# xXJSONDeruloXx/linux-fg

Hardware: AMD Instinct MI355X
Metric: interpolated frames/s, 1080p->4K RGBA8 (higher is better)
Workload: dtype f32 arithmetic on u8 RGBA (u8 in, u8 out; int8 motion vectors); 1 GPU; 1080p->2160p scale+motion(8,16)+interpolate; order=one call per stage, semantics=reference, frames_in_flight=3, content=translated (the motion stage's best case but `static`; see content_sweep), parallelism=one frame pair per GPU x1, gpu_max_hw_queues=4

## Files before the change

### include/linuxfg_hip.h

```cpp
#ifndef LINUXFG_HIP_H
#define LINUXFG_HIP_H

#include <stddef.h>
#include <stdint.h>

#ifdef __cplusplus
extern "C" {
#endif

#define LFG_ABI_VERSION 1

typedef enum lfg_status {
    LFG_OK = 0,
    LFG_ERR_INVALID = -1,
    LFG_ERR_DEVICE = -2,
    LFG_ERR_NOMEM = -3,
    LFG_ERR_UNSUPPORTED = -4
} lfg_status;

typedef enum lfg_format {
    LFG_FORMAT_RGBA8_UNORM = 0,
    LFG_FORMAT_MV_S8X2 = 1,
    LFG_FORMAT_MV_S16X2_Q2 = 2
} lfg_format;

typedef struct lfg_frame {
    void    *data;
    uint32_t width;
    uint32_t height;
    uint32_t pitch;
    uint32_t format;
    uint32_t owned;
    uint32_t reserved;
} lfg_frame;

typedef struct lfg_context lfg_context;
typedef struct lfg_ring lfg_ring;

typedef enum lfg_stage {
    LFG_STAGE_SCALE = 0,
    LFG_STAGE_MOTION = 1,
    LFG_STAGE_INTERPOLATE = 2,
    LFG_STAGE_COUNT = 3
} lfg_stage;


int         lfg_abi_version(void);
int         lfg_device_count(void);

int         lfg_context_create(int device_ordinal, lfg_context **out_ctx);
void        lfg_context_destroy(lfg_context *ctx);
int         lfg_context_set_stream(lfg_context *ctx, void *hip_stream);
void       *lfg_context_get_stream(lfg_context *ctx);
int         lfg_context_device(const lfg_context *ctx);
int         lfg_sync(lfg_context *ctx);

#define LFG_MAX_LANES 4
int         lfg_lanes(lfg_context *ctx, int count);
int         lfg_lane_count(const lfg_context *ctx);
int         lfg_lane_current(const lfg_context *ctx);
int         lfg_lane_select(lfg_context *ctx, int lane);
int         lfg_lane_mark(lfg_context *ctx);
int         lfg_lane_wait(lfg_context *ctx, int other);
int         lfg_lane_sync(lfg_context *ctx);
const char *lfg_last_error(const lfg_context *ctx);


int  lfg_frame_create(lfg_context *ctx, uint32_t width, uint32_t height, uint32_t format, lfg_frame *out);
void lfg_frame_destroy(lfg_context *ctx, lfg_frame *frame);
int  lfg_frame_wrap(void *device_ptr, uint32_t width, uint32_t height, uint32_t pitch, uint32_t format,
                    lfg_frame *out);
int  lfg_frame_copy(lfg_context *ctx, const lfg_frame *src, lfg_frame *dst);

int  lfg_staging_create(lfg_context *ctx, size_t bytes, void **out_host_ptr);
void lfg_staging_destroy(lfg_context *ctx, void *host_ptr);

int  lfg_frame_upload(lfg_context *ctx, lfg_frame *dst, const void *host, size_t bytes);
int  lfg_frame_download(lfg_context *ctx, const lfg_frame *src, void *host, size_t bytes);

int  lfg_ring_create(lfg_context *ctx, uint32_t slots, size_t slot_bytes, lfg_ring **out_ring);
void lfg_ring_destroy(lfg_ring *ring);
int  lfg_ring_acquire(lfg_ring *ring, void **out_host_ptr, uint32_t *out_slot);
int  lfg_ring_upload(lfg_ring *ring, uint32_t slot, lfg_frame *dst);
int  lfg_ring_download(lfg_ring *ring, uint32_t slot, const lfg_frame *src);
int  lfg_ring_wait(lfg_ring *ring, uint32_t slot);
int  lfg_ring_fence_slot(lfg_ring *ring, uint32_t slot);


int  lfg_scale(lfg_context *ctx, const lfg_frame *in, lfg_frame *out);
int  lfg_scale_last_kernel(const lfg_context *ctx);

int  lfg_motion(lfg_context *ctx, const lfg_frame *prev, const lfg_frame *curr, lfg_frame *mv,
                int block_size, float search_radius);

typedef enum lfg_motion_mode { LFG_MOTION_PREFILTERED = 0, LFG_MOTION_EXACT_ONLY = 1 } lfg_motion_mode;
int  lfg_set_motion_mode(lfg_context *ctx, int mode);
int  lfg_motion_last_stats(lfg_context *ctx, uint32_t *out_tiles, uint32_t *out_fallback_tiles,
                           double *out_mean_recorded);
int  lfg_motion_open_segments(lfg_context *ctx, uint32_t *out_open, uint32_t *out_segments);
int  lfg_motion_lean_stats(lfg_context *ctx, int *out_used, uint32_t *out_tiles, uint32_t *out_tiles_left);
int  lfg_motion_strip_stats(lfg_context *ctx, uint32_t *out_rows, uint32_t *out_columns);
int  lfg_motion_last_variant(const lfg_context *ctx);
int  lfg_motion_prediction_stats(const lfg_context *ctx, uint64_t *out_verdicts, uint64_t *out_lean_wrong,
                                 uint64_t *out_grid_wrong, uint64_t *out_second_pass_wrong);
int  lfg_motion_workspace_size(lfg_context *ctx, uint32_t width, uint32_t height, uint64_t *out_bytes);
int  lfg_motion_plan(const lfg_context *ctx, int *out_rim_split, int *out_workgroups);

int  lfg_motion_pyramid(lfg_context *ctx, const lfg_frame *prev, const lfg_frame *curr, lfg_frame *mv,
                        int levels, int coarse_radius, int refine_radius);
typedef enum lfg_motion_estimator { LFG_ESTIMATOR_FULL_SEARCH = 0, LFG_ESTIMATOR_PYRAMID = 1 } lfg_motion_estimator;
int  lfg_set_motion_estimator(lfg_context *ctx, int estimator);

typedef enum lfg_semantics { LFG_SEMANTICS_REFERENCE = 0, LFG_SEMANTICS_INTENDED = 1 } lfg_semantics;
int  lfg_set_semantics(lfg_context *ctx, int semantics);

int  lfg_interpolate(lfg_context *ctx, const lfg_frame *prev, const lfg_frame *curr, const lfg_frame *mv,
                     lfg_frame *out, float factor);

int  lfg_interpolate_frames(lfg_context *ctx, const lfg_frame *prev, const lfg_frame *curr,
                            lfg_frame *out, float factor);

#define LFG_MAX_FACTORS 16
int  lfg_interpolate_multi(lfg_context *ctx, const lfg_frame *prev, const lfg_frame *curr, const lfg_frame *mv,
                           lfg_frame *const *outs, const float *factors, uint32_t count);
int  lfg_set_fused_motion_interpolate(lfg_context *ctx, int enabled);

int  lfg_interpolate_frames_multi(lfg_context *ctx, const lfg_frame *prev, const lfg_frame *curr,
                                  lfg_frame *const *outs, const float *factors, uint32_t count);

int  lfg_interpolate_compensated(lfg_context *ctx, const lfg_frame *prev, const lfg_frame *curr, const lfg_frame *mv,
                                 lfg_frame *out, float factor, int match_sad);
int  lfg_interpolate_compensated_multi(lfg_context *ctx, const lfg_frame *prev, const lfg_frame *curr, const lfg_frame *mv,
                                       lfg_frame *const *outs, const float *factors, uint32_t count, int match_sad);
typedef enum lfg_interpolator { LFG_INTERPOLATOR_SHADER = 0, LFG_INTERPOLATOR_COMPENSATED = 1 } lfg_interpolator;
int  lfg_set_interpolator(lfg_context *ctx, int interpolator, int match_sad);

typedef struct lfg_mask { void *data; uint32_t width, height, pitch; } lfg_mask;
int  lfg_static_mask(lfg_context *ctx, const lfg_frame *prev, const lfg_frame *curr, int tolerance, const lfg_mask *out);
int  lfg_interpolate_compensated_masked(lfg_context *ctx, const lfg_frame *prev, const lfg_frame *curr, const lfg_frame *mv,
                                        const lfg_mask *mask, lfg_frame *out, float factor, int match_sad);
int  lfg_interpolate_compensated_masked_multi(lfg_context *ctx, const lfg_frame *prev, const lfg_frame *curr, const lfg_frame *mv,
                                              const lfg_mask *mask, lfg_frame *const *outs, const float *factors, uint32_t count,
                                              int match_sad);
int  lfg_set_static_protection(lfg_context *ctx, int tolerance);

int  lfg_extrapolate_compensated(lfg_context *ctx, const lfg_frame *prev, const lfg_frame *curr, const lfg_frame *mv,
                                 lfg_frame *out, float ahead, int match_sad);
int  lfg_extrapolate_compensated_multi(lfg_context *ctx, const lfg_frame *prev, const lfg_frame *curr, const lfg_frame *mv,
                                       lfg_frame *const *outs, const float *aheads, uint32_t count, int match_sad);
typedef enum lfg_generation { LFG_GENERATION_INTERPOLATE = 0, LFG_GENERATION_EXTRAPOLATE = 1 } lfg_generation;
int  lfg_set_generation(lfg_context *ctx, int generation);

int  lfg_motion_consistency(lfg_context *ctx, const lfg_frame *a, const lfg_frame *b, int tolerance, const lfg_mask *out);
int  lfg_interpolate_compensated_bidirectional(lfg_context *ctx, const lfg_frame *prev, const lfg_frame *curr, const lfg_frame *fwd,
                                               const lfg_frame *bwd, lfg_frame *out, float factor, int match_sad, int tolerance);
int  lfg_interpolate_compensated_bidirectional_multi(lfg_context *ctx, const lfg_frame *prev, const lfg_frame *curr,
                                                     const lfg_frame *fwd, const lfg_frame *bwd, lfg_frame *const *outs,
                                                     const float *factors, uint32_t count, int match_sad, int tolerance);
int  lfg_set_bidirectional(lfg_context *ctx, int tolerance);

#define LFG_HOLE_REACH_MAX 255
int  lfg_hole_fill_plane(lfg_context *ctx, const lfg_frame *keys, int reach, int pass_static, lfg_frame *plane);
int  lfg_set_hole_reach(lfg_context *ctx, int reach);

int  lfg_motion_refine(lfg_context *ctx, const lfg_frame *prev, const lfg_frame *curr, const lfg_frame *mv_in,
                       lfg_frame *mv_out, int radius);
int  lfg_set_vector_refinement(lfg_context *ctx, int radius);

int  lfg_frame_halve(lfg_context *ctx, const lfg_frame *in, lfg_frame *out);
int  lfg_motion_expand(lfg_context *ctx, const lfg_frame *prev, const lfg_frame *curr, const lfg_frame *mv_low,
                       lfg_frame *mv_out, int radius);
int  lfg_set_half_resolution_motion(lfg_context *ctx, int radius);

int  lfg_motion_subpel(lfg_context *ctx, const lfg_frame *prev, const lfg_frame *curr, const lfg_frame *mv_in,
                       lfg_frame *mvq_out, int radius);
int  lfg_interpolate_compensated_subpel(lfg_context *ctx, const lfg_frame *prev, const lfg_frame *curr, const lfg_frame *mvq,
                                        lfg_frame *out, float factor, int match_sad);
int  lfg_interpolate_compensated_subpel_multi(lfg_context *ctx, const lfg_frame *prev, const lfg_frame *curr, const lfg_frame *mvq,
                                              lfg_frame *const *outs, const float *factors, uint32_t count, int match_sad);
int  lfg_set_subpixel_vectors(lfg_context *ctx, int radius);

typedef struct lfg_pair_stats { uint64_t pixels, matched, sad_sum; } lfg_pair_stats;
int  lfg_pair_match(lfg_context *ctx, const lfg_frame *prev, const lfg_frame *curr, const lfg_frame *mv,
                    int match_sad, void *device_stats );
int  lfg_cut_fallback(lfg_context *ctx, const lfg_frame *prev, const lfg_frame *curr, const void *device_stats,
                      int min_matched_permille, lfg_frame *const *outs, const float *factors, uint32_t count);
int  lfg_set_cut_detection(lfg_context *ctx, int min_matched_permille);
int  lfg_last_pair_stats(lfg_context *ctx, lfg_pair_stats *out_stats, int *out_cut);

typedef struct lfg_frame_diff_stats { uint64_t pixels; uint64_t sse[4]; uint64_t hist[256]; } lfg_frame_diff_stats;
int  lfg_frame_diff(lfg_context *ctx, const lfg_frame *a, const lfg_frame *b, uint32_t channel_mask,
                    int accumulate, void *device_stats );
typedef struct lfg_frame_diff_summary { uint64_t pixels, differing, over_1; uint32_t max_abs, p50, p99; double mse, psnr_db; } lfg_frame_diff_summary;
int  lfg_frame_diff_summarize(const lfg_frame_diff_stats *host_stats, uint32_t channel_mask, lfg_frame_diff_summary *out);

typedef struct lfg_nv12 { void *y; void *uv; uint32_t width, height, y_pitch, uv_pitch; } lfg_nv12;
typedef enum { LFG_YUV_BT601 = 0, LFG_YUV_BT709 = 1 } lfg_yuv_matrix;
typedef enum { LFG_YUV_LIMITED = 0, LFG_YUV_FULL = 1 } lfg_yuv_range;
typedef enum { LFG_CHROMA_REPLICATE = 0, LFG_CHROMA_LEFT = 1 } lfg_chroma_siting;
int  lfg_nv12_to_rgba(lfg_context *ctx, const lfg_nv12 *in, lfg_frame *out, int matrix, int range, int siting);
int  lfg_rgba_to_nv12(lfg_context *ctx, const lfg_frame *in, const lfg_nv12 *out, int matrix, int range, int siting);
int  lfg_yuv_coefficients(int matrix, int range, int32_t to_rgb[5], int32_t to_yuv[9]);

int  lfg_sharpen(lfg_context *ctx, const lfg_frame *in, lfg_frame *out, int strength);

typedef enum {
    LFG_FILTER_NEAREST = 0, LFG_FILTER_BILINEAR = 1, LFG_FILTER_CATMULL_ROM = 2, LFG_FILTER_MITCHELL = 3, LFG_FILTER_LANCZOS2 = 4,
    LFG_FILTER_LANCZOS3 = 5
} lfg_filter;
#define LFG_RESAMPLE_MAX_TAPS 64
int  lfg_resample(lfg_context *ctx, const lfg_frame *in, lfg_frame *out, int filter);
int  lfg_resample_taps(int filter, uint32_t in_size, uint32_t out_size, int32_t *first, uint32_t *count, int16_t *weights);

int  lfg_interpolate_scale(lfg_context *ctx, const lfg_frame *prev, const lfg_frame *curr, const lfg_frame *mv,
                           lfg_frame *out, float factor);
int  lfg_set_fused_interpolate_scale(lfg_context *ctx, int enabled);

int  lfg_mv_export_rgba32f(lfg_context *ctx, const lfg_frame *mv, void *device_rgba32f);


#define LFG_COMM_ID_BYTES 128
typedef struct lfg_comm_id { char bytes[LFG_COMM_ID_BYTES]; } lfg_comm_id;
int  lfg_comm_unique_id(lfg_comm_id *out_id);
int  lfg_comm_init(lfg_context *ctx, int nranks, int rank, const lfg_comm_id *id);
int  lfg_comm_rank(const lfg_context *ctx);
int  lfg_comm_ranks(const lfg_context *ctx);
int  lfg_broadcast_frame(lfg_context *ctx, lfg_frame *frame, int root);
int  lfg_broadcast_frame_lane(lfg_context *ctx, lfg_frame *frame, int root);
int  lfg_comm_wait(lfg_context *ctx);
int  lfg_comm_sync(lfg_context *ctx);
int  lfg_comm_reserved_cus(const lfg_context *ctx);
int  lfg_comm_cu_mask(const lfg_context *ctx, uint32_t *out_words, int words);
int  lfg_comm_probe(lfg_context *ctx, int workgroups, int microseconds, int every_lane );
int  lfg_comm_probe_ms(lfg_context *ctx, float *out_ms);
int  lfg_comm_destroy(lfg_context *ctx);


int  lfg_selftest_sqrt(lfg_context *ctx, uint32_t lo_bits, uint32_t hi_bits, uint64_t *out_mismatches);

int  lfg_diag_scale_2x_strip(uint32_t in_height, uint32_t xcd, uint32_t index, uint32_t *out_strips_per_xcd,
                             int32_t *out_first_step, int32_t *out_steps);


int  lfg_profile_enable(lfg_context *ctx, int enabled);
int  lfg_profile_reset(lfg_context *ctx);
int  lfg_profile_get(lfg_context *ctx, int stage, double *out_total_ms, uint64_t *out_launches);

#ifdef __cplusplus
}
#endif
#endif
```

### linux-fg_amd/capi.py

```python
from __future__ import annotations

import ctypes
import os

import numpy as np

_HERE = os.path.dirname(os.path.abspath(__file__))
LIB_PATH = os.environ.get("LFG_LIB") or os.path.join(_HERE, "liblinuxfg_hip.so")

FORMAT_RGBA8 = 0
FORMAT_MV_S8X2 = 1
FORMAT_MV_S16X2_Q2 = 2
STAGE_SCALE, STAGE_MOTION, STAGE_INTERPOLATE = 0, 1, 2
MOTION_PREFILTERED, MOTION_EXACT_ONLY = 0, 1
SEMANTICS_REFERENCE, SEMANTICS_INTENDED = 0, 1
ESTIMATOR_FULL_SEARCH, ESTIMATOR_PYRAMID = 0, 1
INTERPOLATOR_SHADER, INTERPOLATOR_COMPENSATED = 0, 1
GENERATION_INTERPOLATE, GENERATION_EXTRAPOLATE = 0, 1
DEFAULT_MATCH_SAD = 48
HOLE_REACH_MAX = 255
YUV_BT601, YUV_BT709 = 0, 1
YUV_LIMITED, YUV_FULL = 0, 1
CHROMA_REPLICATE, CHROMA_LEFT = 0, 1
_BPP = {FORMAT_RGBA8: 4, FORMAT_MV_S8X2: 2, FORMAT_MV_S16X2_Q2: 4}
# ... 7 lines not shown

class LfgError(RuntimeError):
    pass


class Frame(ctypes.Structure):
    _fields_ = [("data", ctypes.c_void_p), ("width", ctypes.c_uint32), ("height", ctypes.c_uint32),
                ("pitch", ctypes.c_uint32), ("format", ctypes.c_uint32), ("owned", ctypes.c_uint32),
                ("reserved", ctypes.c_uint32)]


class Nv12(ctypes.Structure):
    _fields_ = [("y", ctypes.c_void_p), ("uv", ctypes.c_void_p), ("width", ctypes.c_uint32), ("height", ctypes.c_uint32),
                ("y_pitch", ctypes.c_uint32), ("uv_pitch", ctypes.c_uint32)]


class Mask(ctypes.Structure):
    _fields_ = [("data", ctypes.c_void_p), ("width", ctypes.c_uint32), ("height", ctypes.c_uint32), ("pitch", ctypes.c_uint32)]


class PairStats(ctypes.Structure):
    _fields_ = [("pixels", ctypes.c_uint64), ("matched", ctypes.c_uint64), ("sad_sum", ctypes.c_uint64)]

    def as_tuple(self):
        return int(self.pixels), int(self.matched), int(self.sad_sum)


class FrameDiffStats(ctypes.Structure):
    _fields_ = [("pixels", ctypes.c_uint64), ("sse", ctypes.c_uint64 * 4), ("hist", ctypes.c_uint64 * 256)]

    def as_tuple(self):
        return int(self.pixels), tuple(int(v) for v in self.sse), tuple(int(v) for v in self.hist)


class FrameDiffSummary(ctypes.Structure):
    _fields_ = [("pixels", ctypes.c_uint64), ("differing", ctypes.c_uint64), ("over_1", ctypes.c_uint64),
                ("max_abs", ctypes.c_uint32), ("p50", ctypes.c_uint32), ("p99", ctypes.c_uint32),
                ("mse", ctypes.c_double), ("psnr_db", ctypes.c_double)]

    def as_dict(self):
        return {name: (float if name in ("mse", "psnr_db") else int)(getattr(self, name)) for name, _ in self._fields_}


_vp, _i, _u32, _sz = ctypes.c_void_p, ctypes.c_int, ctypes.c_uint32, ctypes.c_size_t
_FP = ctypes.POINTER(Frame)

SIGNATURES = {
    "lfg_abi_version": (_i, []),
    "lfg_device_count": (_i, []),
    "lfg_context_create": (_i, [_i, ctypes.POINTER(_vp)]),
    "lfg_context_destroy": (None, [_vp]),
    "lfg_context_set_stream": (_i, [_vp, _vp]),
    "lfg_context_get_stream": (_vp, [_vp]),
    "lfg_context_device": (_i, [_vp]),
    "lfg_sync": (_i, [_vp]),
    "lfg_lanes": (_i, [_vp, _i]),
    "lfg_lane_count": (_i, [_vp]),
    "lfg_lane_current": (_i, [_vp]),
    "lfg_lane_select": (_i, [_vp, _i]),
    "lfg_lane_mark": (_i, [_vp]),
    "lfg_lane_wait": (_i, [_vp, _i]),
    "lfg_lane_sync": (_i, [_vp]),
    "lfg_last_error": (ctypes.c_char_p, [_vp]),
    "lfg_frame_create": (_i, [_vp, _u32, _u32, _u32, _FP]),
    "lfg_frame_destroy": (None, [_vp, _FP]),
    "lfg_frame_wrap": (_i, [_vp, _u32, _u32, _u32, _u32, _FP]),
    "lfg_frame_copy": (_i, [_vp, _FP, _FP]),
    "lfg_staging_create": (_i, [_vp, _sz, ctypes.POINTER(_vp)]),
    "lfg_staging_destroy": (None, [_vp, _vp]),
    "lfg_frame_upload": (_i, [_vp, _FP, _vp, _sz]),
    "lfg_frame_download": (_i, [_vp, _FP, _vp, _sz]),
    "lfg_ring_create": (_i, [_vp, _u32, _sz, ctypes.POINTER(_vp)]),
    "lfg_ring_destroy": (None, [_vp]),
    "lfg_ring_acquire": (_i, [_vp, ctypes.POINTER(_vp), ctypes.POINTER(_u32)]),
    "lfg_ring_upload": (_i, [_vp, _u32, _FP]),
    "lfg_ring_download": (_i, [_vp, _u32, _FP]),
    "lfg_ring_wait": (_i, [_vp, _u32]),
    "lfg_ring_fence_slot": (_i, [_vp, _u32]),
    "lfg_scale": (_i, [_vp, _FP, _FP]),
    "lfg_motion": (_i, [_vp, _FP, _FP, _FP, _i, ctypes.c_float]),
    "lfg_set_motion_mode": (_i, [_vp, _i]),
    "lfg_motion_last_stats": (_i, [_vp, ctypes.POINTER(_u32), ctypes.POINTER(_u32), ctypes.POINTER(ctypes.c_double)]),
    "lfg_motion_open_segments": (_i, [_vp, ctypes.POINTER(_u32), ctypes.POINTER(_u32)]),
    "lfg_motion_lean_stats": (_i, [_vp, ctypes.POINTER(_i), ctypes.POINTER(_u32), ctypes.POINTER(_u32)]),
    "lfg_motion_strip_stats": (_i, [_vp, ctypes.POINTER(_u32), ctypes.POINTER(_u32)]),
    "lfg_motion_prediction_stats": (_i, [_vp] + [ctypes.POINTER(ctypes.c_uint64)] * 4),
    "lfg_motion_workspace_size": (_i, [_vp, _u32, _u32, ctypes.POINTER(ctypes.c_uint64)]),
    "lfg_motion_plan": (_i, [_vp, ctypes.POINTER(_i), ctypes.POINTER(_i)]),
    "lfg_motion_pyramid": (_i, [_vp, _FP, _FP, _FP, _i, _i, _i]),
    "lfg_set_motion_estimator": (_i, [_vp, _i]),
    "lfg_set_semantics": (_i, [_vp, _i]),
    "lfg_interpolate": (_i, [_vp, _FP, _FP, _FP, _FP, ctypes.c_float]),
    "lfg_interpolate_frames": (_i, [_vp, _FP, _FP, _FP, ctypes.c_float]),
    "lfg_interpolate_multi": (_i, [_vp, _FP, _FP, _FP, ctypes.POINTER(_FP), ctypes.POINTER(ctypes.c_float), _u32]),
    "lfg_interpolate_frames_multi": (_i, [_vp, _FP, _FP, ctypes.POINTER(_FP), ctypes.POINTER(ctypes.c_float), _u32]),
    "lfg_interpolate_scale": (_i, [_vp, _FP, _FP, _FP, _FP, ctypes.c_float]),
    "lfg_interpolate_compensated": (_i, [_vp, _FP, _FP, _FP, _FP, ctypes.c_float, _i]),
    "lfg_interpolate_compensated_multi": (_i, [_vp, _FP, _FP, _FP, ctypes.POINTER(_FP), ctypes.POINTER(ctypes.c_float), _u32, _i]),
    "lfg_set_interpolator": (_i, [_vp, _i, _i]),
    "lfg_static_mask": (_i, [_vp, _FP, _FP, _i, ctypes.POINTER(Mask)]),
    "lfg_interpolate_compensated_masked": (_i, [_vp, _FP, _FP, _FP, ctypes.POINTER(Mask), _FP, ctypes.c_float, _i]),
    "lfg_interpolate_compensated_masked_multi": (_i, [_vp, _FP, _FP, _FP, ctypes.POINTER(Mask), ctypes.POINTER(_FP),
                                                      ctypes.POINTER(ctypes.c_float), _u32, _i]),
    "lfg_set_static_protection": (_i, [_vp, _i]),
    "lfg_extrapolate_compensated": (_i, [_vp, _FP, _FP, _FP, _FP, ctypes.c_float, _i]),
    "lfg_extrapolate_compensated_multi": (_i, [_vp, _FP, _FP, _FP, ctypes.POINTER(_FP), ctypes.POINTER(ctypes.c_float), _u32, _i]),
    "lfg_set_generation": (_i, [_vp, _i]),
    "lfg_motion_consistency": (_i, [_vp, _FP, _FP, _i, ctypes.POINTER(Mask)]),
    "lfg_interpolate_compensated_bidirectional": (_i, [_vp, _FP, _FP, _FP, _FP, _FP, ctypes.c_float, _i, _i]),
    "lfg_interpolate_compensated_bidirectional_multi": (_i, [_vp, _FP, _FP, _FP, _FP, ctypes.POINTER(_FP),
                                                             ctypes.POINTER(ctypes.c_float), _u32, _i, _i]),
    "lfg_set_bidirectional": (_i, [_vp, _i]),
    "lfg_hole_fill_plane": (_i, [_vp, _FP, _i, _i, _FP]),
    "lfg_set_hole_reach": (_i, [_vp, _i]),
    "lfg_motion_refine": (_i, [_vp, _FP, _FP, _FP, _FP, _i]),
    "lfg_set_vector_refinement": (_i, [_vp, _i]),
    "lfg_frame_halve": (_i, [_vp, _FP, _FP]),
    "lfg_motion_expand": (_i, [_vp, _FP, _FP, _FP, _FP, _i]),
    "lfg_set_half_resolution_motion": (_i, [_vp, _i]),
    "lfg_motion_subpel": (_i, [_vp, _FP, _FP, _FP, _FP, _i]),
    "lfg_interpolate_compensated_subpel": (_i, [_vp, _FP, _FP, _FP, _FP, ctypes.c_float, _i]),
    "lfg_interpolate_compensated_subpel_multi": (_i, [_vp, _FP, _FP, _FP, ctypes.POINTER(_FP), ctypes.POINTER(ctypes.c_float), _u32, _i]),
    "lfg_set_subpixel_vectors": (_i, [_vp, _i]),
    "lfg_pair_match": (_i, [_vp, _FP, _FP, _FP, _i, _vp]),
    "lfg_cut_fallback": (_i, [_vp, _FP, _FP, _vp, _i, ctypes.POINTER(_FP), ctypes.POINTER(ctypes.c_float), _u32]),
    "lfg_set_cut_detection": (_i, [_vp, _i]),
    "lfg_last_pair_stats": (_i, [_vp, ctypes.POINTER(PairStats), ctypes.POINTER(_i)]),
    "lfg_frame_diff": (_i, [_vp, _FP, _FP, _u32, _i, _vp]),
    "lfg_frame_diff_summarize": (_i, [ctypes.POINTER(FrameDiffStats), _u32, ctypes.POINTER(FrameDiffSummary)]),
    "lfg_nv12_to_rgba": (_i, [_vp, ctypes.POINTER(Nv12), _FP, _i, _i, _i]),
    "lfg_rgba_to_nv12": (_i, [_vp, _FP, ctypes.POINTER(Nv12), _i, _i, _i]),
    "lfg_sharpen": (_i, [_vp, _FP, _FP, _i]),
    "lfg_resample": (_i, [_vp, _FP, _FP, _i]),
    "lfg_resample_taps": (_i, [_i, _u32, _u32, ctypes.POINTER(ctypes.c_int32), ctypes.POINTER(ctypes.c_uint32), ctypes.POINTER(ctypes.c_int16)]),
    "lfg_yuv_coefficients": (_i, [_i, _i, ctypes.POINTER(ctypes.c_int32), ctypes.POINTER(ctypes.c_int32)]),
    "lfg_set_fused_interpolate_scale": (_i, [_vp, _i]),
    "lfg_set_fused_motion_interpolate": (_i, [_vp, _i]),
    "lfg_mv_export_rgba32f": (_i, [_vp, _FP, _vp]),
    "lfg_selftest_sqrt": (_i, [_vp, _u32, _u32, ctypes.POINTER(ctypes.c_uint64)]),
    "lfg_comm_unique_id": (_i, [_vp]),
    "lfg_comm_init": (_i, [_vp, _i, _i, _vp]),
    "lfg_comm_rank": (_i, [_vp]),
    "lfg_comm_ranks": (_i, [_vp]),
    "lfg_broadcast_frame": (_i, [_vp, _FP, _i]),
    "lfg_comm_wait": (_i, [_vp]),
    "lfg_comm_destroy": (_i, [_vp]),
    "lfg_comm_sync": (_i, [_vp]),
    "lfg_comm_reserved_cus": (_i, [_vp]),
    "lfg_comm_cu_mask": (_i, [_vp, ctypes.POINTER(_u32), _i]),
    "lfg_comm_probe": (_i, [_vp, _i, _i, _i]),
    "lfg_broadcast_frame_lane": (_i, [_vp, _FP, _i]),
    "lfg_comm_probe_ms": (_i, [_vp, ctypes.POINTER(ctypes.c_float)]),
    "lfg_motion_last_variant": (_i, [_vp]),
    "lfg_scale_last_kernel": (_i, [_vp]),
    "lfg_diag_scale_2x_strip": (_i, [_u32, _u32, _u32, ctypes.POINTER(_u32), ctypes.POINTER(ctypes.c_int32), ctypes.POINTER(ctypes.c_int32)]),
    "lfg_profile_enable": (_i, [_vp, _i]),
    "lfg_profile_reset": (_i, [_vp]),
    "lfg_profile_get": (_i, [_vp, _i, ctypes.POINTER(ctypes.c_double), ctypes.POINTER(ctypes.c_uint64)]),
}

_lib = None


def summarize(record, channel_mask: int = 0xF) -> dict:
    pixels, sse, hist = record
    s, out = FrameDiffStats(int(pixels), (ctypes.c_uint64 * 4)(*sse), (ctypes.c_uint64 * 256)(*hist)), FrameDiffSummary()
    rc = load().lfg_frame_diff_summarize(ctypes.byref(s), int(channel_mask), ctypes.byref(out))
    if rc != 0:
        raise LfgError(f"lfg_frame_diff_summarize failed ({rc}): bad mask, no pixels, or a histogram that does not sum to them")
    return out.as_dict()


def yuv_coefficients(matrix: int, yuv_range: int):
    to_rgb, to_yuv = (ctypes.c_int32 * 5)(), (ctypes.c_int32 * 9)()
    rc = load().lfg_yuv_coefficients(int(matrix), int(yuv_range), to_rgb, to_yuv)
    if rc != 0:
        raise LfgError(f"lfg_yuv_coefficients failed ({rc}): unknown matrix or range")
    return tuple(int(v) for v in to_rgb), tuple(int(v) for v in to_yuv)


def resample_taps(filt: int, n_in: int, n_out: int):
    n_in, n_out = int(n_in), int(n_out)
    rows = n_out if 0 < n_out < 2 ** 32 else 0
    first, count = np.zeros(rows, np.int32), np.zeros(rows, np.uint32)
    weights = np.zeros((rows, RESAMPLE_MAX_TAPS), np.int16)
    rc = load().lfg_resample_taps(int(filt), n_in if 0 < n_in < 2 ** 32 else 0, rows,
                                  first.ctypes.data_as(ctypes.POINTER(ctypes.c_int32)), count.ctypes.data_as(ctypes.POINTER(ctypes.c_uint32)),
                                  weights.ctypes.data_as(ctypes.POINTER(ctypes.c_int16)))
    if rc != 0:
        err = LfgError(f"lfg_resample_taps failed ({rc}): " + ("more than RESAMPLE_MAX_TAPS taps per sample" if rc == ERR_UNSUPPORTED
                                                                 else "a size of 0 or an unknown filter"))
        err.code = rc
        raise err
    return first, count, weights


def load() -> ctypes.CDLL:
    global _lib
    if _lib is None:
        if not os.path.exists(LIB_PATH):
            raise LfgError(f"{LIB_PATH} not built: run `python -c 'import __graft_entry__ as g; g.build()'` "
                           "(there is no CPU fallback)")
        os.environ.setdefault("GPU_MAX_HW_QUEUES", "8")
        L = ctypes.CDLL(LIB_PATH)
        for name, (res, args) in SIGNATURES.items():
            fn = getattr(L, name)
            fn.restype, fn.argtypes = res, args
        _lib = L
    return _lib


class Context:

    def __init__(self, device: int = 0, stream: int | None = None):
        self.lib = load()
        h = _vp()
        rc = self.lib.lfg_context_create(device, ctypes.byref(h))
        if rc != 0:
            raise LfgError(f"lfg_context_create failed ({rc}): {self.lib.lfg_last_error(None).decode()}")
        self.h = h
        self._frames: list[Frame] = []
        if stream is not None:
            self.set_stream(stream)

    def _check(self, rc: int, what: str):
        if rc != 0:
            raise LfgError(f"{what} failed ({rc}): {self.lib.lfg_last_error(self.h).decode()}")

    def close(self):
        if getattr(self, "h", None):
            for f in self._frames:
                self.lib.lfg_frame_destroy(self.h, ctypes.byref(f))
            self._frames.clear()
            self.lib.lfg_context_destroy(self.h)
            self.h = None

    def __enter__(self):
        return self

    def __exit__(self, *exc):
        self.close()

    def __del__(self):
        try:
            self.close()
        except Exception:
            pass

    def set_stream(self, stream: int | None):
        self._check(self.lib.lfg_context_set_stream(self.h, _vp(stream or 0)), "lfg_context_set_stream")

    def sync(self):
        self._check(self.lib.lfg_sync(self.h), "lfg_sync")

    def lanes(self, count: int):
        self._check(self.lib.lfg_lanes(self.h, int(count)), "lfg_lanes")

    def lane_count(self) -> int:
        return int(self.lib.lfg_lane_count(self.h))

    def lane_current(self) -> int:
        return int(self.lib.lfg_lane_current(self.h))

    def lane_select(self, lane: int):
        self._check(self.lib.lfg_lane_select(self.h, int(lane)), "lfg_lane_select")

    def lane_mark(self):
        self._check(self.lib.lfg_lane_mark(self.h), "lfg_lane_mark")

    def lane_sync(self):
        self._check(self.lib.lfg_lane_sync(self.h), "lfg_lane_sync")

    def lane_wait(self, other: int):
        self._check(self.lib.lfg_lane_wait(self.h, int(other)), "lfg_lane_wait")

    def create_frame(self, width: int, height: int, fmt: int = FORMAT_RGBA8) -> Frame:
        f = Frame()
        self._check(self.lib.lfg_frame_create(self.h, width, height, fmt, ctypes.byref(f)), "lfg_frame_create")
        self._frames.append(f)
        return f

    def destroy_frame(self, f: Frame):
        self.lib.lfg_frame_destroy(self.h, ctypes.byref(f))
        self._frames = [g for g in self._frames if g is not f]

    @staticmethod
    def wrap(device_ptr: int, width: int, height: int, fmt: int = FORMAT_RGBA8, pitch: int | None = None) -> Frame:
        f = Frame()
        rc = load().lfg_frame_wrap(_vp(device_ptr), width, height, pitch or width * _BPP[fmt], fmt, ctypes.byref(f))
        if rc != 0:
            raise LfgError(f"lfg_frame_wrap failed ({rc})")
        return f

    def upload(self, f: Frame, host: np.ndarray):
        a = np.ascontiguousarray(host)
        self._check(self.lib.lfg_frame_upload(self.h, ctypes.byref(f), a.ctypes.data_as(_vp), a.nbytes), "lfg_frame_upload")
        self.sync()

    def download(self, f: Frame) -> np.ndarray:
        if f.format == FORMAT_RGBA8:
            out = np.empty((f.height, f.width, 4), np.uint8)
        elif f.format == FORMAT_MV_S16X2_Q2:
            out = np.empty((f.height, f.width, 2), np.int16)
        else:
            out = np.empty((f.height, f.width, 2), np.int8)
        self._check(self.lib.lfg_frame_download(self.h, ctypes.byref(f), out.ctypes.data_as(_vp), out.nbytes), "lfg_frame_download")
        self.sync()
        return out

    def frame_from(self, host: np.ndarray, fmt: int = FORMAT_RGBA8) -> Frame:
        if fmt == FORMAT_MV_S16X2_Q2 and (host.dtype != np.int16 or host.shape[2:] != (2,)):
            raise LfgError(f"frame_from: FORMAT_MV_S16X2_Q2 takes (H, W, 2) int16, not {host.shape} {host.dtype}")
        f = self.create_frame(host.shape[1], host.shape[0], fmt)
        self.upload(f, host)
        return f

    def copy(self, src: Frame, dst: Frame):
        self._check(self.lib.lfg_frame_copy(self.h, ctypes.byref(src), ctypes.byref(dst)), "lfg_frame_copy")

    def staging_create(self, nbytes: int) -> np.ndarray:
        p = _vp()
        self._check(self.lib.lfg_staging_create(self.h, nbytes, ctypes.byref(p)), "lfg_staging_create")
        a = np.ctypeslib.as_array((ctypes.c_uint8 * nbytes).from_address(p.value))
        self._staging = getattr(self, "_staging", {})
        self._staging[a.ctypes.data] = p.value
        return a

    def staging_destroy(self, a: np.ndarray):
        self.lib.lfg_staging_destroy(self.h, _vp(self._staging.pop(a.ctypes.data)))

    def upload_async(self, f: Frame, host: np.ndarray):
        self._check(self.lib.lfg_frame_upload(self.h, ctypes.byref(f), host.ctypes.data_as(_vp), host.nbytes), "lfg_frame_upload")

    def download_async(self, f: Frame, host: np.ndarray):
        self._check(self.lib.lfg_frame_download(self.h, ctypes.byref(f), host.ctypes.data_as(_vp), host.nbytes), "lfg_frame_download")

    def mv_export_rgba32f(self, mv: Frame) -> np.ndarray:
        tmp = self.create_frame(mv.width * 4, mv.height)
        self._check(self.lib.lfg_mv_export_rgba32f(self.h, ctypes.byref(mv), _vp(tmp.data)), "lfg_mv_export_rgba32f")
        raw = self.download(tmp)
        self.destroy_frame(tmp)
        return raw.reshape(mv.height, mv.width * 16).view(np.float32).reshape(mv.height, mv.width, 4)

    def scale(self, src: Frame, dst: Frame):
        self._check(self.lib.lfg_scale(self.h, ctypes.byref(src), ctypes.byref(dst)), "lfg_scale")

    def motion(self, prev: Frame, curr: Frame, mv: Frame, block_size: int = 8, search_radius: float = 16.0):
        self._check(self.lib.lfg_motion(self.h, ctypes.byref(prev), ctypes.byref(curr), ctypes.byref(mv),
                                        block_size, search_radius), "lfg_motion")

    def set_motion_mode(self, mode: int):
        self._check(self.lib.lfg_set_motion_mode(self.h, mode), "lfg_set_motion_mode")

    def motion_pyramid(self, prev: Frame, curr: Frame, mv: Frame, levels: int = 2, coarse_radius: int = 16, refine_radius: int = 2):
        self._check(self.lib.lfg_motion_pyramid(self.h, ctypes.byref(prev), ctypes.byref(curr), ctypes.byref(mv),
                                                int(levels), int(coarse_radius), int(refine_radius)), "lfg_motion_pyramid")

    def set_motion_estimator(self, estimator: int):
        self._check(self.lib.lfg_set_motion_estimator(self.h, int(estimator)), "lfg_set_motion_estimator")

    def set_semantics(self, semantics: int):
        self._check(self.lib.lfg_set_semantics(self.h, semantics), "lfg_set_semantics")

    def motion_last_stats(self):
        t, f, m = ctypes.c_uint32(), ctypes.c_uint32(), ctypes.c_double()
        self._check(self.lib.lfg_motion_last_stats(self.h, ctypes.byref(t), ctypes.byref(f), ctypes.byref(m)), "lfg_motion_last_stats")
        return t.value, f.value, m.value

    def motion_open_segments(self):
        a, b = ctypes.c_uint32(), ctypes.c_uint32()
        self._check(self.lib.lfg_motion_open_segments(self.h, ctypes.byref(a), ctypes.byref(b)), "lfg_motion_open_segments")
        return a.value, b.value

    def motion_lean_stats(self):
        u, t, l = ctypes.c_int(), ctypes.c_uint32(), ctypes.c_uint32()
        self._check(self.lib.lfg_motion_lean_stats(self.h, ctypes.byref(u), ctypes.byref(t), ctypes.byref(l)), "lfg_motion_lean_stats")
        return bool(u.value), t.value, l.value

    def motion_strip_stats(self):
        a, b = ctypes.c_uint32(), ctypes.c_uint32()
        self._check(self.lib.lfg_motion_strip_stats(self.h, ctypes.byref(a), ctypes.byref(b)), "lfg_motion_strip_stats")
        return a.value, b.value

    def motion_prediction_stats(self):
        v = [ctypes.c_uint64() for _ in range(4)]
        self._check(self.lib.lfg_motion_prediction_stats(self.h, *[ctypes.byref(x) for x in v]), "lfg_motion_prediction_stats")
        return tuple(int(x.value) for x in v)

    def motion_workspace_size(self, width: int, height: int) -> int:
        n = ctypes.c_uint64()
        self._check(self.lib.lfg_motion_workspace_size(self.h, width, height, ctypes.byref(n)), "lfg_motion_workspace_size")
        return n.value

    def scale_last_kernel(self) -> int:
        return int(self.lib.lfg_scale_last_kernel(self.h))

    def motion_last_variant(self) -> int:
        return int(self.lib.lfg_motion_last_variant(self.h))

    def motion_plan(self):
        a, b = ctypes.c_int(), ctypes.c_int()
        self._check(self.lib.lfg_motion_plan(self.h, ctypes.byref(a), ctypes.byref(b)), "lfg_motion_plan")
        return a.value, b.value

    def interpolate(self, prev: Frame, curr: Frame, mv: Frame, out: Frame, factor: float = 0.5):
        self._check(self.lib.lfg_interpolate(self.h, ctypes.byref(prev), ctypes.byref(curr), ctypes.byref(mv),
                                             ctypes.byref(out), factor), "lfg_interpolate")

    def interpolate_frames(self, prev: Frame, curr: Frame, out: Frame, factor: float = 0.5):
        self._check(self.lib.lfg_interpolate_frames(self.h, ctypes.byref(prev), ctypes.byref(curr),
                                                    ctypes.byref(out), factor), "lfg_interpolate_frames")

    @staticmethod
    def _multi_args(outs, factors):
        n = len(outs)
        if n != len(factors):
            raise ValueError("one output frame per factor")
        return (_FP * n)(*[ctypes.pointer(o) for o in outs]), (ctypes.c_float * n)(*factors), n

    def interpolate_multi(self, prev: Frame, curr: Frame, mv: Frame, outs, factors):
        po, pf, n = self._multi_args(outs, factors)
        self._check(self.lib.lfg_interpolate_multi(self.h, ctypes.byref(prev), ctypes.byref(curr), ctypes.byref(mv), po, pf, n),
                    "lfg_interpolate_multi")

    def interpolate_frames_multi(self, prev: Frame, curr: Frame, outs, factors):
        po, pf, n = self._multi_args(outs, factors)
        self._check(self.lib.lfg_interpolate_frames_multi(self.h, ctypes.byref(prev), ctypes.byref(curr), po, pf, n),
                    "lfg_interpolate_frames_multi")

    def interpolate_compensated(self, prev: Frame, curr: Frame, mv: Frame, out: Frame, factor: float = 0.5,
                                match_sad: int = DEFAULT_MATCH_SAD):
        self._check(self.lib.lfg_interpolate_compensated(self.h, ctypes.byref(prev), ctypes.byref(curr), ctypes.byref(mv),
                                                         ctypes.byref(out), factor, int(match_sad)), "lfg_interpolate_compensated")

    def interpolate_compensated_multi(self, prev: Frame, curr: Frame, mv: Frame, outs, factors, match_sad: int = DEFAULT_MATCH_SAD):
        po, pf, n = self._multi_args(outs, factors)
        self._check(self.lib.lfg_interpolate_compensated_multi(self.h, ctypes.byref(prev), ctypes.byref(curr), ctypes.byref(mv),
                                                               po, pf, n, int(match_sad)), "lfg_interpolate_compensated_multi")

    def set_interpolator(self, interpolator: int, match_sad: int = DEFAULT_MATCH_SAD):
        self._check(self.lib.lfg_set_interpolator(self.h, int(interpolator), int(match_sad)), "lfg_set_interpolator")

    _MASK_ROW = 4096

    def create_mask(self, width: int, height: int, pitch: int | None = None, offset: int = 0, fill: int = 0):
        pitch = width if pitch is None else int(pitch)
        rows = -(-(offset + pitch * height) // self._MASK_ROW)
        f = self.frame_from(np.full((rows, self._MASK_ROW // 4, 4), fill, np.uint8))
        return f, Mask(f.data + offset, width, height, pitch)

    def mask_from(self, host: np.ndarray, pitch: int | None = None, offset: int = 0, fill: int = 0):
        h, w = host.shape
        f, m = self.create_mask(w, h, pitch, offset, fill)
        raw = np.full(f.height * self._MASK_ROW, fill, np.uint8)
        rows = raw[offset:offset + m.pitch * h].reshape(h, m.pitch)
        rows[:, :w] = host
        self.upload(f, raw.reshape(f.height, -1, 4))
        return f, m

    def download_mask(self, f: Frame, m: Mask):
        raw = self.download(f).reshape(-1)
        offset = m.data - f.data
        return raw[offset:offset + m.pitch * m.height].reshape(m.height, m.pitch), raw

    def static_mask(self, prev: Frame, curr: Frame, mask: Mask, tolerance: int = 0):
        self._check(self.lib.lfg_static_mask(self.h, ctypes.byref(prev), ctypes.byref(curr), int(tolerance), ctypes.byref(mask)),
                    "lfg_static_mask")

    def interpolate_compensated_masked(self, prev: Frame, curr: Frame, mv: Frame, mask: Mask, out: Frame, factor: float = 0.5,
                                       match_sad: int = DEFAULT_MATCH_SAD):
        self._check(self.lib.lfg_interpolate_compensated_masked(self.h, ctypes.byref(prev), ctypes.byref(curr), ctypes.byref(mv),
                                                                ctypes.byref(mask), ctypes.byref(out), factor, int(match_sad)),
                    "lfg_interpolate_compensated_masked")

    def interpolate_compensated_masked_multi(self, prev: Frame, curr: Frame, mv: Frame, mask: Mask, outs, factors,
                                             match_sad: int = DEFAULT_MATCH_SAD):
        po, pf, n = self._multi_args(outs, factors)
        self._check(self.lib.lfg_interpolate_compensated_masked_multi(self.h, ctypes.byref(prev), ctypes.byref(curr), ctypes.byref(mv),
                                                                      ctypes.byref(mask), po, pf, n, int(match_sad)),
                    "lfg_interpolate_compensated_masked_multi")

    def set_static_protection(self, tolerance: int):
        self._check(self.lib.lfg_set_static_protection(self.h, int(tolerance)), "lfg_set_static_protection")

    def extrapolate_compensated(self, prev: Frame, curr: Frame, mv: Frame, out: Frame, ahead: float = 1.0,
                                match_sad: int = DEFAULT_MATCH_SAD):
        self._check(self.lib.lfg_extrapolate_compensated(self.h, ctypes.byref(prev), ctypes.byref(curr), ctypes.byref(mv),
                                                         ctypes.byref(out), ahead, int(match_sad)), "lfg_extrapolate_compensated")

    def extrapolate_compensated_multi(self, prev: Frame, curr: Frame, mv: Frame, outs, aheads, match_sad: int = DEFAULT_MATCH_SAD):
        po, pf, n = self._multi_args(outs, aheads)
        self._check(self.lib.lfg_extrapolate_compensated_multi(self.h, ctypes.byref(prev), ctypes.byref(curr), ctypes.byref(mv),
                                                               po, pf, n, int(match_sad)), "lfg_extrapolate_compensated_multi")

    def set_generation(self, generation: int):
        self._check(self.lib.lfg_set_generation(self.h, int(generation)), "lfg_set_generation")

    def motion_consistency(self, a: Frame, b: Frame, tolerance: int, out: Mask):
        self._check(self.lib.lfg_motion_consistency(self.h, ctypes.byref(a), ctypes.byref(b), int(tolerance), ctypes.byref(out)),
                    "lfg_motion_consistency")

    def interpolate_compensated_bidirectional(self, prev: Frame, curr: Frame, fwd: Frame, bwd: Frame, out: Frame, factor: float = 0.5,
                                              match_sad: int = DEFAULT_MATCH_SAD, tolerance: int = 1):
        self._check(self.lib.lfg_interpolate_compensated_bidirectional(
            self.h, ctypes.byref(prev), ctypes.byref(curr), ctypes.byref(fwd), ctypes.byref(bwd), ctypes.byref(out), factor,
            int(match_sad), int(tolerance)), "lfg_interpolate_compensated_bidirectional")

    def interpolate_compensated_bidirectional_multi(self, prev: Frame, curr: Frame, fwd: Frame, bwd: Frame, outs, factors,
                                                    match_sad: int = DEFAULT_MATCH_SAD, tolerance: int = 1):
        po, pf, n = self._multi_args(outs, factors)
        self._check(self.lib.lfg_interpolate_compensated_bidirectional_multi(
            self.h, ctypes.byref(prev), ctypes.byref(curr), ctypes.byref(fwd), ctypes.byref(bwd), po, pf, n, int(match_sad),
            int(tolerance)), "lfg_interpolate_compensated_bidirectional_multi")

    def set_bidirectional(self, tolerance: int):
        self._check(self.lib.lfg_set_bidirectional(self.h, int(tolerance)), "lfg_set_bidirectional")

    def hole_fill_plane(self, keys: Frame, plane: Frame, reach: int, pass_static: bool = False):
        self._check(self.lib.lfg_hole_fill_plane(self.h, ctypes.byref(keys), int(reach), int(bool(pass_static)), ctypes.byref(plane)),
                    "lfg_hole_fill_plane")

    def set_hole_reach(self, reach: int):
        self._check(self.lib.lfg_set_hole_reach(self.h, int(reach)), "lfg_set_hole_reach")

    def motion_refine(self, prev: Frame, curr: Frame, mv_in: Frame, mv_out: Frame, radius: int = 1):
        self._check(self.lib.lfg_motion_refine(self.h, ctypes.byref(prev), ctypes.byref(curr), ctypes.byref(mv_in),
                                               ctypes.byref(mv_out), int(radius)), "lfg_motion_refine")

    def set_vector_refinement(self, radius: int):
        self._check(self.lib.lfg_set_vector_refinement(self.h, int(radius)), "lfg_set_vector_refinement")

    def frame_halve(self, src: Frame, dst: Frame):
        self._check(self.lib.lfg_frame_halve(self.h, ctypes.byref(src), ctypes.byref(dst)), "lfg_frame_halve")

    def motion_expand(self, prev: Frame, curr: Frame, mv_low: Frame, mv_out: Frame, radius: int = 1):
        self._check(self.lib.lfg_motion_expand(self.h, ctypes.byref(prev), ctypes.byref(curr), ctypes.byref(mv_low),
                                               ctypes.byref(mv_out), int(radius)), "lfg_motion_expand")

    def motion_subpel(self, prev: Frame, curr: Frame, mv_in: Frame, mvq_out: Frame, radius: int = 1):
        self._check(self.lib.lfg_motion_subpel(self.h, ctypes.byref(prev), ctypes.byref(curr), ctypes.byref(mv_in),
                                               ctypes.byref(mvq_out), int(radius)), "lfg_motion_subpel")

    def interpolate_compensated_subpel(self, prev: Frame, curr: Frame, mvq: Frame, out: Frame, factor: float = 0.5,
                                       match_sad: int = DEFAULT_MATCH_SAD):
        self._check(self.lib.lfg_interpolate_compensated_subpel(self.h, ctypes.byref(prev), ctypes.byref(curr), ctypes.byref(mvq),
                                                                ctypes.byref(out), factor, int(match_sad)), "lfg_interpolate_compensated_subpel")

    def interpolate_compensated_subpel_multi(self, prev: Frame, curr: Frame, mvq: Frame, outs, factors, match_sad: int = DEFAULT_MATCH_SAD):
        po, pf, n = self._multi_args(outs, factors)
        self._check(self.lib.lfg_interpolate_compensated_subpel_multi(self.h, ctypes.byref(prev), ctypes.byref(curr), ctypes.byref(mvq),
                                                                      po, pf, n, int(match_sad)), "lfg_interpolate_compensated_subpel_multi")

# ... 151 lines not shown
```

### linux-fg_amd/csrc/interpolate.hip

```cpp
#include "lfg_device.hpp"
#include "lfg_internal.hpp"
#include "lfg_interp.hpp"

namespace lfg {

constexpr int kRsrcRgba8Unorm = (int)(4u | (5u << 3) | (6u << 6) | (7u << 9) | (0u << 12) | (10u << 15));

__device__ __forceinline__ uint32_t mix_pack(const V4 p, const V4 c, float t) {
    return pack_rgba8_unorm(mixf(p.x, c.x, t), mixf(p.y, c.y, t), mixf(p.z, c.z, t), mixf(p.w, c.w, t));
}

struct RowTaps { bool below; float w00, w10; };

__device__ __forceinline__ float uv_of(int p, int size, float rcp, int rcpExact, const float *__restrict__ table) {
#ifdef LFG_DIAG_UV_TABLE
    return table[p];
#endif
    if (!rcpExact) return table[p];
    const float x = (float)p + 0.5f, q0 = x * rcp;
    return __builtin_fmaf(__builtin_fmaf(-q0, (float)size, x), rcp, q0);
}

__device__ __forceinline__ float uv_div(int p, int size) { return ((float)p + 0.5f) / (float)size; }

__device__ __forceinline__ RowTaps row_taps(int p, int W, float uvx) {
    const float pk = (float)p;
    const float u = uvx * (float)W - 0.5f;
    const float fu = __builtin_floorf(u);
    const float a = u - fu;
    return RowTaps{fu < pk, (1.0f - a) * (1.0f - 0.0f), a * (1.0f - 0.0f)};
}

__device__ __forceinline__ V4 row_blend(const RowTaps &t, const f32x4 left, const f32x4 mid, const f32x4 right) {
    const f32x4 t00 = t.below ? left : mid, t10 = t.below ? mid : right;
    return V4{t.w00 * t00.x + t.w10 * t10.x, t.w00 * t00.y + t.w10 * t10.y, t.w00 * t00.z + t.w10 * t10.z, t.w00 * t00.w + t.w10 * t10.w};
}

struct QuadRows { uint32_t t[2][6]; };

__device__ __forceinline__ V4 cell_blend(const RowTaps &tx, const RowTaps &ty, const QuadRows &q, int i) {
    const float w00 = tx.w00 * ty.w00, w10 = tx.w10 * ty.w00, w01 = tx.w00 * ty.w10, w11 = tx.w10 * ty.w10;
    const V4 t00 = unorm4(tx.below ? q.t[0][i] : q.t[0][i + 1]), t10 = unorm4(tx.below ? q.t[0][i + 1] : q.t[0][i + 2]);
    const V4 t01 = unorm4(tx.below ? q.t[1][i] : q.t[1][i + 1]), t11 = unorm4(tx.below ? q.t[1][i + 1] : q.t[1][i + 2]);
    V4 r;
    r.x = ((w00 * t00.x + w10 * t10.x) + w01 * t01.x) + w11 * t11.x;
    r.y = ((w00 * t00.y + w10 * t10.y) + w01 * t01.y) + w11 * t11.y;
    r.z = ((w00 * t00.z + w10 * t10.z) + w01 * t01.z) + w11 * t11.z;
    r.w = ((w00 * t00.w + w10 * t10.w) + w01 * t01.w) + w11 * t11.w;
    return r;
}

__device__ __forceinline__ QuadRows load_quad_rows(const uint8_t *__restrict__ img, int pitch, int W, int r0, int r1, int px0, bool edges) {
    const uint8_t *a = img + (size_t)r0 * (size_t)pitch, *b = img + (size_t)r1 * (size_t)pitch;
    const uint4 qa = *reinterpret_cast<const uint4 *>(a + (size_t)px0 * 4u), qb = *reinterpret_cast<const uint4 *>(b + (size_t)px0 * 4u);
    QuadRows q;
    q.t[0][0] = q.t[0][5] = q.t[1][0] = q.t[1][5] = 0u;
    if (edges) {
        const size_t xl = (size_t)max(px0 - 1, 0) * 4u, xr = (size_t)min(px0 + 4, W - 1) * 4u;
        q.t[0][0] = *reinterpret_cast<const uint32_t *>(a + xl); q.t[0][5] = *reinterpret_cast<const uint32_t *>(a + xr);
        q.t[1][0] = *reinterpret_cast<const uint32_t *>(b + xl); q.t[1][5] = *reinterpret_cast<const uint32_t *>(b + xr);
    }
    q.t[0][1] = qa.x; q.t[0][2] = qa.y; q.t[0][3] = qa.z; q.t[0][4] = qa.w;
    q.t[1][1] = qb.x; q.t[1][2] = qb.y; q.t[1][3] = qb.z; q.t[1][4] = qb.w;
    return q;
}

template <bool INTENDED>
__device__ __forceinline__ bool pixel_taps(const uint8_t *__restrict__ prev, int prevPitch, const uint8_t *__restrict__ curr, int currPitch,
                                           int W, int H, int8_t mxi, int8_t myi, float uvx, float uvy, float t, SampleTaps &sp, SampleTaps &sc) {
    float mx = (float)mxi, my = (float)myi;
    if (INTENDED) { mx = mx / (float)W; my = my / (float)H; }
    if (!sample_inside(uvx, uvy, mx, my, -t) && !sample_inside(uvx, uvy, mx, my, 1.0f - t)) return false;
    sp = sample_taps(prev, W, H, prevPitch, uvx, uvy, mx, my, -t);
    sc = sample_taps(curr, W, H, currPitch, uvx, uvy, mx, my, 1.0f - t);
    return sp.inside || sc.inside;
}

__device__ __forceinline__ uint32_t pixel_finish(const SampleTaps &sp, const SampleTexels &tp, const SampleTaps &sc, const SampleTexels &tc, float t) {
    const V4 p = sample_finish(sp, tp);
    const V4 c = sample_finish(sc, tc);
    return pack_rgba8_unorm(mixf(p.x, c.x, t), mixf(p.y, c.y, t), mixf(p.z, c.z, t), mixf(p.w, c.w, t));
}

__device__ __forceinline__ bool row_is_centre(const InterpTables &tb, int py) {
    const int row = __builtin_amdgcn_readfirstlane(py);
    const uint32_t w = reinterpret_cast<const uint32_t *>(tb.centreY)[row >> 2];
    return ((w >> (8 * (row & 3))) & 1u) != 0u;
}

static bool fast_frames(const lfg_frame &prev, const lfg_frame &curr, const lfg_frame &mv) {
    const auto small = [](const lfg_frame &f) { return (uint64_t)f.pitch * f.height < (1ull << 31); };
    return small(prev) && small(curr) && (uintptr_t)prev.data % 4u == 0 && (uintptr_t)curr.data % 4u == 0 &&
           mv.pitch % 8u == 0 && (uintptr_t)mv.data % 8u == 0;
}
static bool fast_output(const lfg_frame &o) { return o.pitch % 16u == 0 && (uintptr_t)o.data % 16u == 0; }

#ifndef LFG_INTERP_WAVES
#define LFG_INTERP_WAVES 6
#endif
#ifndef LFG_INTERP_WAVES_MULTI
#define LFG_INTERP_WAVES_MULTI 6
#endif
constexpr int kMaxMulti = 4;
struct MultiTargets {
    uint8_t *out[kMaxMulti];
    int pitch[kMaxMulti];
    float t[kMaxMulti];
};

template <int N, bool INTENDED>
__global__ __launch_bounds__(256, N == 1 ? LFG_INTERP_WAVES : LFG_INTERP_WAVES_MULTI) void interpolate_kernel(
    const uint8_t *__restrict__ prev, int prevPitch, const uint8_t *__restrict__ curr, int currPitch,
    const int8_t *__restrict__ mv, int mvPitch, MultiTargets tg, int W, int H, bool wideStores,
    InterpTables tb, int fast) {
    const int lane = threadIdx.x & 63;
    const int py = blockIdx.y * 4 + (threadIdx.x >> 6);
    if (py >= H) return;
    const int px0 = (blockIdx.x * 64 + lane) * 4;
    if (px0 >= W) return;
#ifdef LFG_DIAG_INTERP_ROWS_CENTRE
    const bool rowCentre = fast;
#else
    const bool rowCentre = fast && row_is_centre(tb, py);
#endif
    const int8_t *mrow = mv + (size_t)py * (size_t)mvPitch;
    const bool full = (px0 + 3 < W) && ((mvPitch & 7) == 0) && wideStores;

    int8_t m[8];
    uint32_t o[N][4];
    bool zero = false;
    if (full) {
        const uint2 mm = *reinterpret_cast<const uint2 *>(mrow + (size_t)px0 * 2u);
        zero = (mm.x | mm.y) == 0u;
        if (rowCentre && zero) {
            const __amdgpu_buffer_rsrc_t rP = __builtin_amdgcn_make_buffer_rsrc(const_cast<uint8_t *>(prev), 0, H * prevPitch, kRsrcRgba8Unorm);
            const __amdgpu_buffer_rsrc_t rC = __builtin_amdgcn_make_buffer_rsrc(const_cast<uint8_t *>(curr), 0, H * currPitch, kRsrcRgba8Unorm);
            const int offP = py * prevPitch + px0 * 4, offC = py * currPitch + px0 * 4;
            f32x4 tp[6], tc[6];
#pragma unroll
            for (int i = 0; i < 4; ++i) tp[i + 1] = buffer_load_rgba8_format(rP, offP + 4 * i, 0);
#pragma unroll
            for (int i = 0; i < 4; ++i) tc[i + 1] = buffer_load_rgba8_format(rC, offC + 4 * i, 0);
#ifdef LFG_DIAG_INTERP_NO_PATCH
            const bool laneGood = true;
#else
            const bool laneGood = ((tb.goodMask[blockIdx.x] >> lane) & 1ull) != 0ull;
#endif
            V4 fp[4], fc[4];
            if (laneGood) {
#pragma unroll
                for (int i = 0; i < 4; ++i) { fp[i] = V4{tp[i + 1].x, tp[i + 1].y, tp[i + 1].z, tp[i + 1].w}; fc[i] = V4{tc[i + 1].x, tc[i + 1].y, tc[i + 1].z, tc[i + 1].w}; }
            } else {
                const int xl = max(px0 - 1, 0) * 4, xr = min(px0 + 4, W - 1) * 4;
                tp[0] = buffer_load_rgba8_format(rP, py * prevPitch + xl, 0); tp[5] = buffer_load_rgba8_format(rP, py * prevPitch + xr, 0);
                tc[0] = buffer_load_rgba8_format(rC, py * currPitch + xl, 0); tc[5] = buffer_load_rgba8_format(rC, py * currPitch + xr, 0);
#pragma unroll
                for (int i = 0; i < 4; ++i) {
                    const RowTaps t = row_taps(px0 + i, W, uv_div(px0 + i, W));
                    fp[i] = row_blend(t, tp[i], tp[i + 1], tp[i + 2]);
                    fc[i] = row_blend(t, tc[i], tc[i + 1], tc[i + 2]);
                }
            }
#pragma unroll
            for (int k = 0; k < N; ++k) {
#pragma unroll
                for (int i = 0; i < 4; ++i) o[k][i] = mix_pack(fp[i], fc[i], tg.t[k]);
                *reinterpret_cast<uint4 *>(tg.out[k] + (size_t)py * (size_t)tg.pitch[k] + (size_t)px0 * 4u) = uint4{o[k][0], o[k][1], o[k][2], o[k][3]};
            }
            return;
        }
        if (fast && zero) {
            const bool laneGood = ((tb.goodMask[blockIdx.x] >> lane) & 1ull) != 0ull;
            const RowTaps ty = row_taps(py, H, uv_div(py, H));
            const int j0 = ty.below ? py - 1 : py;
            const int r0 = clampi(j0, 0, H - 1), r1 = clampi(j0 + 1, 0, H - 1);
            const QuadRows qp = load_quad_rows(prev, prevPitch, W, r0, r1, px0, !laneGood);
            const QuadRows qc = load_quad_rows(curr, currPitch, W, r0, r1, px0, !laneGood);
            V4 fp[4], fc[4];
#pragma unroll
            for (int i = 0; i < 4; ++i) {
                RowTaps tx = RowTaps{false, 1.0f, 0.0f};
                if (!laneGood) tx = row_taps(px0 + i, W, uv_div(px0 + i, W));
                fp[i] = cell_blend(tx, ty, qp, i);
                fc[i] = cell_blend(tx, ty, qc, i);
            }
#pragma unroll
            for (int k = 0; k < N; ++k) {
#pragma unroll
                for (int i = 0; i < 4; ++i) o[k][i] = mix_pack(fp[i], fc[i], tg.t[k]);
                *reinterpret_cast<uint4 *>(tg.out[k] + (size_t)py * (size_t)tg.pitch[k] + (size_t)px0 * 4u) = uint4{o[k][0], o[k][1], o[k][2], o[k][3]};
            }
            return;
        }
        m[0] = (int8_t)(mm.x & 0xff); m[1] = (int8_t)((mm.x >> 8) & 0xff);
        m[2] = (int8_t)((mm.x >> 16) & 0xff); m[3] = (int8_t)(mm.x >> 24);
        m[4] = (int8_t)(mm.y & 0xff); m[5] = (int8_t)((mm.y >> 8) & 0xff);
        m[6] = (int8_t)((mm.y >> 16) & 0xff); m[7] = (int8_t)(mm.y >> 24);
#ifdef LFG_DIAG_MV_UNIFORM
        {
            const int8_t *centre = mv + (size_t)(H / 2) * (size_t)mvPitch + (size_t)(W / 2) * 2u;
            const int8_t cx = centre[0], cy = centre[1];
#pragma unroll
            for (int i = 0; i < 4; ++i) { m[2 * i] = cx; m[2 * i + 1] = cy; }
            zero = (cx | cy) == 0;
        }
#endif
    } else {
#pragma unroll
        for (int i = 0; i < 4; ++i) {
            const int px = min(px0 + i, W - 1);
            m[2 * i] = mrow[(size_t)px * 2u]; m[2 * i + 1] = mrow[(size_t)px * 2u + 1];
        }
    }

#ifndef LFG_INTERP_SURE_OUT
#define LFG_INTERP_SURE_OUT 1
#endif
    if (LFG_INTERP_SURE_OUT && !INTENDED && !zero) {
        bool allOut = true;
#pragma unroll
        for (int k = 0; k < N; ++k) {
            const float t = tg.t[k], sa = -t, sb = 1.0f - t;
#pragma unroll
            for (int i = 0; i < 4; ++i) {
                const float mx = (float)m[2 * i], my = (float)m[2 * i + 1];
                const bool outA = __builtin_fabsf(mx * sa) >= 1.0f || __builtin_fabsf(my * sa) >= 1.0f;
                const bool outB = __builtin_fabsf(mx * sb) >= 1.0f || __builtin_fabsf(my * sb) >= 1.0f;
                allOut = allOut && outA && outB;
            }
        }
        if (allOut) {
#pragma unroll
            for (int k = 0; k < N; ++k) {
                uint8_t *orow = tg.out[k] + (size_t)py * (size_t)tg.pitch[k];
                if (full) {
                    *reinterpret_cast<uint4 *>(orow + (size_t)px0 * 4u) = uint4{0u, 0u, 0u, 0u};
                } else {
                    for (int i = 0; i < 4 && px0 + i < W; ++i) *reinterpret_cast<uint32_t *>(orow + (size_t)(px0 + i) * 4u) = 0u;
                }
            }
            return;
        }
    }
    const float uvy = uv_of(py, H, tb.rcpH, tb.rcpExact, tb.uvy);
    float uvxOf[4];
#pragma unroll
    for (int i = 0; i < 4; ++i) uvxOf[i] = uv_of(min(px0 + i, W - 1), W, tb.rcpW, tb.rcpExact, tb.uvx);
#pragma unroll
    for (int i = 0; i < 4; ++i) {
        const bool still = m[2 * i] == 0 && m[2 * i + 1] == 0;
        SampleTaps sp, sc;
        SampleTexels tp, tc;
#pragma unroll
        for (int k = 0; k < N; ++k) {
            const float t = tg.t[k];
            if (k == 0 || !still) {
                o[k][i] = 0u;
                if (!pixel_taps<INTENDED>(prev, prevPitch, curr, currPitch, W, H, m[2 * i], m[2 * i + 1], uvxOf[i], uvy, t, sp, sc)) continue;
                tp = sample_load(sp); tc = sample_load(sc);
            }
            o[k][i] = pixel_finish(sp, tp, sc, tc, t);
        }
    }
#pragma unroll
    for (int k = 0; k < N; ++k) {
        uint8_t *orow = tg.out[k] + (size_t)py * (size_t)tg.pitch[k];
        if (full) {
            *reinterpret_cast<uint4 *>(orow + (size_t)px0 * 4u) = uint4{o[k][0], o[k][1], o[k][2], o[k][3]};
        } else {
            for (int i = 0; i < 4 && px0 + i < W; ++i)
                *reinterpret_cast<uint32_t *>(orow + (size_t)(px0 + i) * 4u) = o[k][i];
        }
    }
}

template <int N>
static void launch_n(hipStream_t s, dim3 grid, const lfg_frame &prev, const lfg_frame &curr, const lfg_frame &mv,
                     const MultiTargets &tg, int W, int H, bool wide, bool intended, const InterpTables &tb, int fast) {
    if (intended)
        hipLaunchKernelGGL((interpolate_kernel<N, true>), grid, dim3(256), 0, s,
                           (const uint8_t *)prev.data, (int)prev.pitch, (const uint8_t *)curr.data, (int)curr.pitch,
                           (const int8_t *)mv.data, (int)mv.pitch, tg, W, H, wide, tb, fast);
    else
        hipLaunchKernelGGL((interpolate_kernel<N, false>), grid, dim3(256), 0, s,
                           (const uint8_t *)prev.data, (int)prev.pitch, (const uint8_t *)curr.data, (int)curr.pitch,
                           (const int8_t *)mv.data, (int)mv.pitch, tg, W, H, wide, tb, fast);
}

hipError_t launch_interpolate_multi(hipStream_t s, const lfg_frame &prev, const lfg_frame &curr, const lfg_frame &mv,
                                    const lfg_frame *const *outs, const float *factors, int count, bool intended,
                                    const InterpTables &tb) {
    const int W = (int)curr.width, H = (int)curr.height;
    const int quads = (W + 3) / 4;
    const dim3 grid((quads + 63) / 64, (H + 3) / 4);
    for (int first = 0; first < count; first += kMaxMulti) {
        const int n = count - first < kMaxMulti ? count - first : kMaxMulti;
        MultiTargets tg{};
        bool wide = true;
        for (int k = 0; k < kMaxMulti; ++k) {
            const lfg_frame &o = *outs[first + (k < n ? k : 0)];
            tg.out[k] = (uint8_t *)o.data; tg.pitch[k] = (int)o.pitch; tg.t[k] = factors[first + (k < n ? k : 0)];
            wide = wide && fast_output(o);
        }
        const int fast = fast_frames(prev, curr, mv) && wide && tb.goodMask && W < (1 << 20) && H < (1 << 20) ? 1 : 0;
        switch (n) {
            case 1: launch_n<1>(s, grid, prev, curr, mv, tg, W, H, wide, intended, tb, fast); break;
            case 2: launch_n<2>(s, grid, prev, curr, mv, tg, W, H, wide, intended, tb, fast); break;
            case 3: launch_n<3>(s, grid, prev, curr, mv, tg, W, H, wide, intended, tb, fast); break;
            default: launch_n<4>(s, grid, prev, curr, mv, tg, W, H, wide, intended, tb, fast); break;
        }
        hipError_t e = hipGetLastError();
        if (e != hipSuccess) return e;
    }
    return hipSuccess;
}

hipError_t launch_interpolate(hipStream_t s, const lfg_frame &prev, const lfg_frame &curr,
                              const lfg_frame &mv, const lfg_frame &out, float factor, bool intended, const InterpTables &tb) {
    const lfg_frame *outs[1] = {&out};
    return launch_interpolate_multi(s, prev, curr, mv, outs, &factor, 1, intended, tb);
}

__global__ __launch_bounds__(256) void mv_export_kernel(const int8_t *__restrict__ mv, int mvPitch,
                                                        float4 *__restrict__ out, int W, int H) {
    const int px = blockIdx.x * 64 + (threadIdx.x & 63);
    const int py = blockIdx.y * 4 + (threadIdx.x >> 6);
    if (px >= W || py >= H) return;
    const int8_t *m = mv + (size_t)py * (size_t)mvPitch + (size_t)px * 2u;
    out[(size_t)py * (size_t)W + (size_t)px] = float4{(float)m[0], (float)m[1], 0.0f, 1.0f};
}

hipError_t launch_mv_export(hipStream_t s, const lfg_frame &mv, float *rgba32f) {
    dim3 grid((mv.width + 63) / 64, (mv.height + 3) / 4);
    hipLaunchKernelGGL(mv_export_kernel, grid, dim3(256), 0, s, (const int8_t *)mv.data, (int)mv.pitch,
                       reinterpret_cast<float4 *>(rgba32f), (int)mv.width, (int)mv.height);
    return hipGetLastError();
}

}
```

### linux-fg_amd/csrc/lfg_capi.cpp

```cpp
#include <algorithm>
#include <cmath>
#include <cstdio>
#include <cstdlib>
#include <cstring>
#include <new>

#include "lfg_internal.hpp"

#define LFG_EXPORT extern "C" __attribute__((visibility("default")))

namespace {

std::string g_create_error;

int fail(lfg_context *ctx, int code, const std::string &msg) {
    if (ctx) ctx->error = msg; else g_create_error = msg;
    return code;
}

int fail_hip(lfg_context *ctx, hipError_t e, const char *what) {
    return fail(ctx, e == hipErrorOutOfMemory ? LFG_ERR_NOMEM : LFG_ERR_DEVICE,
                std::string(what) + ": " + hipGetErrorString(e));
}

// ... 229 lines not shown
        cur.motion_ws_layout.rimSplit2 == rimSplit2) return LFG_OK;
    lfg::MotionWorkspaceLayout layout;
    if (ctx->motion_slots == 0) {
        ctx->motion_slots = lfg::prefilter_slots();
        if (ctx->knobs.debug) fprintf(stderr, "lfg: motion prefilter: %d workgroups resident at once\n", ctx->motion_slots);
    }
    const size_t bytes = lfg::motion_workspace_bytes(width, height, ctx->motion_slots, rimSplit, rimSplit2, &layout);
    if (bytes > cur.motion_ws_bytes) {
        LFG_HIP(ctx, hipStreamSynchronize(cur.stream));
        if (cur.motion_ws) (void)hipFree(cur.motion_ws);
        cur.motion_ws = nullptr; cur.motion_ws_bytes = 0; cur.motion_ws_w = cur.motion_ws_h = 0;
        LFG_HIP(ctx, hipMalloc((void **)&cur.motion_ws, bytes));
        cur.motion_ws_bytes = bytes;
    } else {
        LFG_HIP(ctx, hipStreamSynchronize(cur.stream));
    }
    const lfg::PrefilterPlanHost plan = lfg::prefilter_plan(width, height, ctx->motion_slots, rimSplit);
    std::vector<uint32_t> tables;
    tables.insert(tables.end(), plan.unitMap.begin(), plan.unitMap.end());
    tables.insert(tables.end(), plan.unitAux.begin(), plan.unitAux.end());
    tables.insert(tables.end(), plan.tileMap.begin(), plan.tileMap.end());
    LFG_HIP(ctx, hipMemcpy(cur.motion_ws + layout.plan, tables.data(), tables.size() * sizeof(uint32_t), hipMemcpyHostToDevice));
    if (rimSplit2) {
        const lfg::PrefilterPlanHost plan2 = lfg::prefilter_plan(width, height, ctx->motion_slots, rimSplit2);
        std::vector<uint32_t> t2;
        t2.insert(t2.end(), plan2.unitMap.begin(), plan2.unitMap.end());
        t2.insert(t2.end(), plan2.unitAux.begin(), plan2.unitAux.end());
        t2.insert(t2.end(), plan2.tileMap.begin(), plan2.tileMap.end());
        LFG_HIP(ctx, hipMemcpy(cur.motion_ws + layout.plan2, t2.data(), t2.size() * sizeof(uint32_t), hipMemcpyHostToDevice));
        if (!plan2.leanTiles.empty()) {
            std::vector<uint32_t> listed = plan2.leanTiles;
            listed.insert(listed.end(), plan2.leanPartial.begin(), plan2.leanPartial.end());
            LFG_HIP(ctx, hipMemcpy(cur.motion_ws + layout.leanTiles, listed.data(), listed.size() * sizeof(uint32_t), hipMemcpyHostToDevice));
        }
    }
    LFG_HIP(ctx, hipMemset(cur.motion_ws + layout.tileFlags, 0, layout.order - layout.tileFlags));
    LFG_HIP(ctx, hipMemset(cur.motion_ws + layout.merge, 0xFF, layout.mergeBytes));
    cur.motion_units = plan.units;
    layout.lastLean = 0;
    cur.motion_ws_layout = layout;
    cur.motion_ws_w = width; cur.motion_ws_h = height;
    return LFG_OK;
}


struct StageTimer {
    lfg_context *ctx;
    hipEvent_t b = nullptr, e = nullptr;
    int stage;
    StageTimer(lfg_context *c, int st) : ctx(c), stage(st) {
        if (!ctx->profile) return;
        if (!ctx->prof_free.empty()) { b = ctx->prof_free.back().first; e = ctx->prof_free.back().second; ctx->prof_free.pop_back(); }
        else if (hipEventCreate(&b) != hipSuccess || hipEventCreate(&e) != hipSuccess) { b = e = nullptr; return; }
        (void)hipEventRecord(b, ctx->cur().stream);
    }
    ~StageTimer() {
        if (!b) return;
        (void)hipEventRecord(e, ctx->cur().stream);
        lfg::ProfileSlot s; s.begin = b; s.end = e; s.stage = stage;
        ctx->prof_pending.push_back(s);
    }
};

int drain_profile(lfg_context *ctx) {
    if (ctx->prof_pending.empty()) return LFG_OK;
    LFG_HIP(ctx, sync_lanes(ctx));
    for (auto &s : ctx->prof_pending) {
        float ms = 0.f;
        if (hipEventElapsedTime(&ms, s.begin, s.end) == hipSuccess) { ctx->prof_ms[s.stage] += ms; ctx->prof_n[s.stage] += 1; }
        ctx->prof_free.emplace_back(s.begin, s.end);
    }
    ctx->prof_pending.clear();
    return LFG_OK;
}

}

struct lfg_ring {
    lfg_context *ctx = nullptr;
    uint32_t slots = 0;
    size_t slot_bytes = 0;
    uint8_t *base = nullptr;
    std::vector<hipEvent_t> done;
    std::vector<uint8_t> busy;
    uint32_t next = 0;
    hipStream_t copy = nullptr;
    hipEvent_t ready = nullptr;
};


hipError_t lfg_own_stream_create(const lfg_context *ctx, hipStream_t *out) {
    if (!ctx || ctx->comm_cus <= 0) return hipStreamCreateWithFlags(out, hipStreamNonBlocking);
    int cus = 0;
    hipError_t e = hipDeviceGetAttribute(&cus, hipDeviceAttributeMultiprocessorCount, ctx->device);
    if (e != hipSuccess) return e;
    if (cus <= ctx->comm_cus) return hipErrorInvalidValue;
    std::vector<uint32_t> mask((size_t)(cus + 31) / 32, 0xffffffffu);
    if (cus % 32) mask.back() = (1u << (cus % 32)) - 1u;
    for (int i = 0; i < ctx->comm_cus; ++i) mask[(size_t)i / 32] &= ~(1u << (i % 32));
    return hipExtStreamCreateWithCUMask(out, (uint32_t)mask.size(), mask.data());
}

int lfg_restream(lfg_context *ctx) {
    LFG_HIP(ctx, hipSetDevice(ctx->device));
    auto again = [&](hipStream_t &own, hipStream_t &used) -> hipError_t {
        if (!own) return hipSuccess;
        hipError_t e = hipStreamSynchronize(own);
        hipStream_t fresh = nullptr;
        if (e == hipSuccess) e = lfg_own_stream_create(ctx, &fresh);
        if (e != hipSuccess) return e;
        (void)hipStreamDestroy(own);
        if (used == own) used = fresh;
        own = fresh;
        return hipSuccess;
    };
    for (size_t k = 0; k < ctx->lanes.size(); ++k) {
        lfg_lane_state &l = ctx->from_selected(k);
        LFG_HIP(ctx, again(l.own_stream, l.stream));
    }
    return LFG_OK;
}

LFG_EXPORT int lfg_abi_version(void) { return LFG_ABI_VERSION; }

LFG_EXPORT int lfg_device_count(void) {
    int n = 0;
    if (hipGetDeviceCount(&n) != hipSuccess) return 0;
    return n;
}

LFG_EXPORT int lfg_context_create(int device_ordinal, lfg_context **out_ctx) {
    if (!out_ctx) return fail(nullptr, LFG_ERR_INVALID, "lfg_context_create: out_ctx is NULL");
    *out_ctx = nullptr;
    int n = 0;
    hipError_t e = hipGetDeviceCount(&n);
    if (e != hipSuccess || n <= 0)
        return fail(nullptr, LFG_ERR_DEVICE, std::string("lfg_context_create: no HIP device (") +
                                                 (e != hipSuccess ? hipGetErrorString(e) : "count 0") + "); there is no CPU fallback");
    const int dev = device_ordinal < 0 ? 0 : device_ordinal;
    if (dev >= n) return fail(nullptr, LFG_ERR_INVALID, "lfg_context_create: device ordinal out of range");
    LFG_HIP(nullptr, hipSetDevice(dev));
    lfg_context *ctx = new (std::nothrow) lfg_context();
    if (!ctx) return fail(nullptr, LFG_ERR_NOMEM, "lfg_context_create: out of host memory");
    ctx->device = dev;
    (void)hipDeviceGetAttribute(&ctx->device_cus, hipDeviceAttributeMultiprocessorCount, dev);
    lfg_lane_state lane0;
    e = lfg_own_stream_create(ctx, &lane0.own_stream);
    if (e != hipSuccess) { delete ctx; return fail_hip(nullptr, e, "hipStreamCreate"); }
    lane0.stream = lane0.own_stream;
    ctx->lanes.push_back(lane0);
    ctx->tables.reserve(17);
    if (const char *m = getenv("LFG_MOTION_HINTS")) ctx->motion_hints = atoi(m) != 0;
    if (const char *m = getenv("LFG_MOTION_LEAN")) ctx->motion_lean = atoi(m) != 0;
    if (const char *m = getenv("LFG_MOTION_RIM_SPLIT")) { const int v = atoi(m); if (v == 4 || v == 8 || v == 48) ctx->rim_split_env = v; }
    if (const char *m = getenv("LFG_FUSED_INTERPOLATE_SCALE")) ctx->fuse_interpolate_scale = atoi(m) != 0;
    if (const char *m = getenv("LFG_FUSED_MOTION_INTERPOLATE")) ctx->fuse_motion_interpolate = atoi(m) != 0;
    if (const char *m = getenv("LFG_MOTION_MODE")) ctx->motion_mode = atoi(m) == 1 ? LFG_MOTION_EXACT_ONLY : LFG_MOTION_PREFILTERED;
    if (const char *m = getenv("LFG_LEAN_FORCE")) ctx->knobs.leanForce = atoi(m) & 1;
    if (getenv("LFG_FALLBACK_FULL")) ctx->knobs.fallbackFull = 1;
    if (const char *m = getenv("LFG_DYN_PARTS_RT")) ctx->knobs.dynParts = atoi(m);
    if (const char *m = getenv("LFG_PREF_GROUPS")) ctx->knobs.prefGroups = atoi(m);
    if (const char *m = getenv("LFG_RESOLVE_GROUPS")) ctx->knobs.resolveGroups = atoi(m);
    if (const char *m = getenv("LFG_MOTION_STRIP")) ctx->knobs.strips = atoi(m) != 0;
    if (const char *m = getenv("LFG_STRIP_PAD")) ctx->knobs.stripPad = atoi(m);
    if (getenv("LFG_DEBUG")) ctx->knobs.debug = 1;
    if (getenv("LFG_DEBUG_DYN")) ctx->knobs.debugDyn = 1;
    if (const char *m = getenv("LFG_DEBUG_DYN_DEEP")) ctx->knobs.debugDynDeep = atoi(m);
    if (const char *m = getenv("LFG_TIER_FORCE")) ctx->knobs.tierForce = atoi(m) & 1;
    if (const char *m = getenv("LFG_FILL_BAND")) { const int v = atoi(m); if (v >= 8 && v <= 1024) ctx->knobs.fillBand = v; }
    if (const char *m = getenv("LFG_COMM_CUS")) { const int v = atoi(m); if (v == 0 || v == 8 || v == 16 || v == 24 || v == 32) ctx->knobs.commCus = v; }
    *out_ctx = ctx;
    return LFG_OK;
}

namespace {
void lane_release(lfg_lane_state &l) {
    if (l.stream) (void)hipStreamSynchronize(l.stream);
    if (l.own_stream && l.own_stream != l.stream) (void)hipStreamSynchronize(l.own_stream);
    for (lfg_frame *f : {&l.mv_tmp, &l.mv_refined, &l.mv_bwd, &l.mv_bwd_refined, &l.half_prev, &l.half_curr, &l.mv_half, &l.mvq_tmp, &l.mid_tmp})
        if (f->data && f->owned) (void)hipFree(f->data);
    if (l.motion_ws) (void)hipFree(l.motion_ws);
    if (l.pyramid_ws) (void)hipFree(l.pyramid_ws);
    if (l.mc_keys) (void)hipFree(l.mc_keys);
    if (l.mc_fill) (void)hipFree(l.mc_fill);
    if (l.static_mask) (void)hipFree(l.static_mask);
    if (l.mcq_keys) (void)hipFree(l.mcq_keys);
    if (l.mark) (void)hipEventDestroy(l.mark);
    if (l.verdict.event) (void)hipEventDestroy(l.verdict.event);
    if (l.verdict.pinned) (void)hipHostFree(l.verdict.pinned);
    if (l.cut.event) (void)hipEventDestroy(l.cut.event);
    if (l.cut.pinned) (void)hipHostFree(l.cut.pinned);
    if (l.cut.device) (void)hipFree(l.cut.device);
    if (l.own_stream) (void)hipStreamDestroy(l.own_stream);
    l = lfg_lane_state{};
}
}

LFG_EXPORT void lfg_context_destroy(lfg_context *ctx) {
    if (!ctx) return;
    (void)hipSetDevice(ctx->device);
    (void)lfg_comm_destroy(ctx);
    (void)sync_lanes(ctx);
    for (auto &l : ctx->lanes) lane_release(l);
    for (auto &s : ctx->prof_pending) { (void)hipEventDestroy(s.begin); (void)hipEventDestroy(s.end); }
    for (auto &p : ctx->prof_free) { (void)hipEventDestroy(p.first); (void)hipEventDestroy(p.second); }
    for (auto &t : ctx->tables) { (void)hipFree(t.d_start); (void)hipFree(t.d_weight); (void)hipFree(t.d_class); (void)hipFree(t.d_palette); }
    for (auto &t : ctx->uv_tables) (void)hipFree(t.d_uv);
    for (auto &t : ctx->resample_tables) (void)hipFree(t.d_base);
    if (ctx->motion_tables) (void)hipFree(ctx->motion_tables);
    delete ctx;
}

LFG_EXPORT int lfg_context_set_stream(lfg_context *ctx, void *hip_stream) {
    if (!ctx) return LFG_ERR_INVALID;
    int rc = drain_profile(ctx);
    if (rc != LFG_OK) return rc;
    LFG_HIP(ctx, hipStreamSynchronize(ctx->cur().stream));
    ctx->cur().stream = hip_stream ? (hipStream_t)hip_stream : ctx->cur().own_stream;
    return LFG_OK;
}

LFG_EXPORT void *lfg_context_get_stream(lfg_context *ctx) { return ctx ? (void *)ctx->cur().stream : nullptr; }


LFG_EXPORT int lfg_lanes(lfg_context *ctx, int count) {
    if (!ctx) return LFG_ERR_INVALID;
    if (count < 1 || count > LFG_MAX_LANES) return fail(ctx, LFG_ERR_INVALID, "lfg_lanes: count must be 1 .. LFG_MAX_LANES");
    LFG_HIP(ctx, hipSetDevice(ctx->device));
    if (ctx->lane >= count) ctx->lane = 0;
    while ((int)ctx->lanes.size() > count) { lane_release(ctx->lanes.back()); ctx->lanes.pop_back(); }
    while ((int)ctx->lanes.size() < count) {
        lfg_lane_state l;
        hipError_t e = lfg_own_stream_create(ctx, &l.own_stream);
        if (e != hipSuccess) return fail_hip(ctx, e, "hipStreamCreate (lane)");
        l.stream = l.own_stream;
        ctx->lanes.push_back(l);
    }
    return LFG_OK;
}

LFG_EXPORT int lfg_lane_count(const lfg_context *ctx) { return ctx ? (int)ctx->lanes.size() : 0; }
LFG_EXPORT int lfg_lane_current(const lfg_context *ctx) { return ctx ? ctx->lane : -1; }

LFG_EXPORT int lfg_lane_select(lfg_context *ctx, int lane) {
    if (!ctx) return LFG_ERR_INVALID;
    if (lane < 0 || lane >= (int)ctx->lanes.size()) return fail(ctx, LFG_ERR_INVALID, "lfg_lane_select: no such lane (lfg_lanes first)");
    ctx->lane = lane;
    return LFG_OK;
}

LFG_EXPORT int lfg_lane_mark(lfg_context *ctx) {
    if (!ctx) return LFG_ERR_INVALID;
    LFG_HIP(ctx, hipSetDevice(ctx->device));
    if (!ctx->cur().mark) LFG_HIP(ctx, hipEventCreateWithFlags(&ctx->cur().mark, hipEventDisableTiming));
    LFG_HIP(ctx, hipEventRecord(ctx->cur().mark, ctx->cur().stream));
    ctx->cur().marked = true;
    return LFG_OK;
}

LFG_EXPORT int lfg_lane_wait(lfg_context *ctx, int other) {
    if (!ctx) return LFG_ERR_INVALID;
    if (other < 0 || other >= (int)ctx->lanes.size()) return fail(ctx, LFG_ERR_INVALID, "lfg_lane_wait: no such lane");
    if (other == ctx->lane) return LFG_OK;
    const lfg_lane_state &o = ctx->lanes[(size_t)other];
    if (!o.marked) return LFG_OK;
    LFG_HIP(ctx, hipStreamWaitEvent(ctx->cur().stream, o.mark, 0));
    return LFG_OK;
}

LFG_EXPORT int lfg_lane_sync(lfg_context *ctx) {
    if (!ctx) return LFG_ERR_INVALID;
    LFG_HIP(ctx, hipSetDevice(ctx->device));
    LFG_HIP(ctx, hipStreamSynchronize(ctx->cur().stream));
    return LFG_OK;
}

LFG_EXPORT int lfg_context_device(const lfg_context *ctx) { return ctx ? ctx->device : -1; }

LFG_EXPORT int lfg_sync(lfg_context *ctx) {
    if (!ctx) return LFG_ERR_INVALID;
    LFG_HIP(ctx, sync_lanes(ctx));
    return LFG_OK;
}

LFG_EXPORT const char *lfg_last_error(const lfg_context *ctx) { return ctx ? ctx->error.c_str() : g_create_error.c_str(); }


LFG_EXPORT int lfg_frame_create(lfg_context *ctx, uint32_t width, uint32_t height, uint32_t format, lfg_frame *out) {
    if (!ctx || !out) return fail(ctx, LFG_ERR_INVALID, "lfg_frame_create: NULL argument");
    const uint32_t bpp = bytes_per_pixel(format);
    if (!bpp || width == 0 || height == 0 || width > 32768u || height > 32768u)
        return fail(ctx, LFG_ERR_INVALID, "lfg_frame_create: bad size or format");
    LFG_HIP(ctx, hipSetDevice(ctx->device));
    void *p = nullptr;
    const size_t bytes = (size_t)width * (size_t)height * (size_t)bpp;
    LFG_HIP(ctx, hipMalloc(&p, bytes));
    out->data = p; out->width = width; out->height = height; out->pitch = width * bpp;
    out->format = format; out->owned = 1; out->reserved = 0;
    return LFG_OK;
}

LFG_EXPORT void lfg_frame_destroy(lfg_context *ctx, lfg_frame *frame) {
    if (!frame) return;
    if (frame->data && frame->owned) {
        if (ctx) { (void)hipSetDevice(ctx->device); (void)sync_lanes(ctx); }
        (void)hipFree(frame->data);
    }
    frame->data = nullptr; frame->width = frame->height = frame->pitch = 0; frame->owned = 0;
}

LFG_EXPORT int lfg_frame_wrap(void *device_ptr, uint32_t width, uint32_t height, uint32_t pitch, uint32_t format,
                              lfg_frame *out) {
    const uint32_t bpp = bytes_per_pixel(format);
    if (!out || !device_ptr || !bpp || width == 0 || height == 0 || pitch < width * bpp) return LFG_ERR_INVALID;
    out->data = device_ptr; out->width = width; out->height = height; out->pitch = pitch;
    out->format = format; out->owned = 0; out->reserved = 0;
    return LFG_OK;
}

LFG_EXPORT int lfg_frame_copy(lfg_context *ctx, const lfg_frame *src, lfg_frame *dst) {
    if (!ctx || !src || !dst || !src->data || !dst->data) return fail(ctx, LFG_ERR_INVALID, "lfg_frame_copy: NULL frame");
    if (!same_size(src, dst) || src->format != dst->format)
        return fail(ctx, LFG_ERR_INVALID, "Source and destination frame dimensions do not match");
    const size_t row = (size_t)src->width * bytes_per_pixel(src->format);
    LFG_HIP(ctx, hipMemcpy2DAsync(dst->data, dst->pitch, src->data, src->pitch, row, src->height,
                                  hipMemcpyDeviceToDevice, ctx->cur().stream));
    return LFG_OK;
}

LFG_EXPORT int lfg_staging_create(lfg_context *ctx, size_t bytes, void **out_host_ptr) {
    if (!ctx || !out_host_ptr || bytes == 0) return fail(ctx, LFG_ERR_INVALID, "lfg_staging_create: bad argument");
    LFG_HIP(ctx, hipSetDevice(ctx->device));
    LFG_HIP(ctx, hipHostMalloc(out_host_ptr, bytes, hipHostMallocDefault));
    return LFG_OK;
}

LFG_EXPORT void lfg_staging_destroy(lfg_context *ctx, void *host_ptr) {
    if (!host_ptr) return;
    if (ctx) (void)sync_lanes(ctx);
    (void)hipHostFree(host_ptr);
}

LFG_EXPORT int lfg_frame_upload(lfg_context *ctx, lfg_frame *dst, const void *host, size_t bytes) {
    if (!ctx || !dst || !dst->data || !host) return fail(ctx, LFG_ERR_INVALID, "lfg_frame_upload: NULL argument");
    const size_t row = (size_t)dst->width * bytes_per_pixel(dst->format);
// ... 274 lines not shown
    if (!out_open || !out_segments) return fail(ctx, LFG_ERR_INVALID, "lfg_motion_open_segments: NULL argument");
    if (!cur.motion_ws || cur.motion_ws_w == 0) return fail(ctx, LFG_ERR_INVALID, "lfg_motion_open_segments: the prefiltered path has not run");
    LFG_HIP(ctx, hipStreamSynchronize(cur.stream));
    const uint32_t tx = (cur.motion_ws_w + 55u) / 56u, ty = (cur.motion_ws_h + 63u) / 64u;
    uint32_t open = 0;
    LFG_HIP(ctx, hipMemcpy(&open, cur.motion_ws + cur.motion_ws_layout.ctrl + lfg::kCtrlOpenCount * sizeof(uint32_t), sizeof(uint32_t), hipMemcpyDeviceToHost));
    *out_open = open;
    *out_segments = tx * ty * 4u;
    return LFG_OK;
}

LFG_EXPORT int lfg_motion_lean_stats(lfg_context *ctx, int *out_used, uint32_t *out_tiles, uint32_t *out_tiles_left) {
    if (!ctx) return LFG_ERR_INVALID;
    lfg_lane_state &cur = ctx->cur();
    if (!out_used || !out_tiles || !out_tiles_left) return fail(ctx, LFG_ERR_INVALID, "lfg_motion_lean_stats: NULL argument");
    if (!cur.motion_ws || cur.motion_ws_w == 0) return fail(ctx, LFG_ERR_INVALID, "lfg_motion_lean_stats: the prefiltered path has not run");
    LFG_HIP(ctx, hipStreamSynchronize(cur.stream));
    uint32_t left = 0;
    LFG_HIP(ctx, hipMemcpy(&left, cur.motion_ws + cur.motion_ws_layout.ctrl + lfg::kCtrlHardCount * sizeof(uint32_t), sizeof(uint32_t), hipMemcpyDeviceToHost));
    *out_used = cur.motion_ws_layout.lastLean;
    *out_tiles = (uint32_t)cur.motion_ws_layout.leanCount;
    *out_tiles_left = cur.motion_ws_layout.lastLean ? left : 0u;
    return LFG_OK;
}

LFG_EXPORT int lfg_motion_strip_stats(lfg_context *ctx, uint32_t *out_rows, uint32_t *out_columns) {
    if (!ctx) return LFG_ERR_INVALID;
    lfg_lane_state &cur = ctx->cur();
    if (!out_rows || !out_columns) return fail(ctx, LFG_ERR_INVALID, "lfg_motion_strip_stats: NULL argument");
    if (!cur.motion_ws || cur.motion_ws_w == 0) return fail(ctx, LFG_ERR_INVALID, "lfg_motion_strip_stats: the prefiltered path has not run");
    LFG_HIP(ctx, hipStreamSynchronize(cur.stream));
    std::vector<uint32_t> t((size_t)cur.motion_ws_h + cur.motion_ws_w);
    LFG_HIP(ctx, hipMemcpy(t.data(), cur.motion_ws + cur.motion_ws_layout.colBand, t.size() * 4, hipMemcpyDeviceToHost));
    uint32_t rows = 0, cols = 0;
    for (uint32_t y = 0; y < cur.motion_ws_h; ++y) rows += t[y] != 0u;
    for (uint32_t x = 0; x < cur.motion_ws_w; ++x) cols += t[cur.motion_ws_h + x] != 0u;
    *out_rows = rows; *out_columns = cols;
    return LFG_OK;
}

LFG_EXPORT int lfg_motion_prediction_stats(const lfg_context *ctx, uint64_t *out_verdicts, uint64_t *out_lean_wrong,
                                           uint64_t *out_grid_wrong, uint64_t *out_second_pass_wrong) {
    if (!ctx) return LFG_ERR_INVALID;
    if (out_verdicts) *out_verdicts = ctx->pred_verdicts;
    if (out_lean_wrong) *out_lean_wrong = ctx->pred_lean_wrong;
    if (out_grid_wrong) *out_grid_wrong = ctx->pred_grid_wrong;
    if (out_second_pass_wrong) *out_second_pass_wrong = ctx->pred_second_wrong;
    return LFG_OK;
}

LFG_EXPORT int lfg_motion_last_stats(lfg_context *ctx, uint32_t *out_tiles, uint32_t *out_fallback_tiles,
                                     double *out_mean_recorded) {
    if (!ctx) return LFG_ERR_INVALID;
    lfg_lane_state &cur = ctx->cur();
    if (!cur.motion_ws || cur.motion_ws_w == 0) return fail(ctx, LFG_ERR_INVALID, "lfg_motion_last_stats: the prefiltered path has not run");
    LFG_HIP(ctx, hipStreamSynchronize(cur.stream));
    const uint32_t tx = (cur.motion_ws_w + 63u) / 64u, ty = (cur.motion_ws_h + 63u) / 64u;
    std::vector<uint32_t> flags((size_t)tx * ty);
    LFG_HIP(ctx, hipMemcpy(flags.data(), cur.motion_ws + cur.motion_ws_layout.tileFlags, flags.size() * 4, hipMemcpyDeviceToHost));
    uint32_t fb = 0;
    for (uint32_t f : flags) fb += f != 0u;
    if (ctx->knobs.debug) {
        uint32_t handed[2] = {0, 0};
        LFG_HIP(ctx, hipMemcpy(handed, cur.motion_ws + cur.motion_ws_layout.queueCount, 8, hipMemcpyDeviceToHost));
        fprintf(stderr, "lfg: motion prefilter: %u requests to hand a segment over (room for %d), %u tiles flagged for the exact kernel\n",
                handed[0], cur.motion_ws_layout.queueCap, handed[1]);
        uint32_t lean[2] = {0, 0};
        LFG_HIP(ctx, hipMemcpy(lean, cur.motion_ws + cur.motion_ws_layout.ctrl + lfg::kCtrlLeanSettled * sizeof(uint32_t), 8, hipMemcpyDeviceToHost));
        uint32_t flags[3] = {0, 0, 0};
        LFG_HIP(ctx, hipMemcpy(flags, cur.motion_ws + cur.motion_ws_layout.orderFlags, 12, hipMemcpyDeviceToHost));
        fprintf(stderr, "lfg: lean kernel: %d tiles listed, %u segments settled, %u left to the generic kernel (counted in -DLFG_LEAN_STATS builds); order flags: hand-over %u, hints %u, lean %u (sample blocks with a close match %u, with an exact one %u)\n",
                cur.motion_ws_layout.leanCount, lean[0], lean[1], flags[0], flags[1], lfg::verdict_lean(flags[2]) ? 1u : 0u, lfg::verdict_close(flags[2]), lfg::verdict_exact(flags[2]));
    }
    if (ctx->knobs.debugDyn) {
        uint32_t handed[2] = {0, 0};
        LFG_HIP(ctx, hipMemcpy(handed, cur.motion_ws + cur.motion_ws_layout.queueCount, 8, hipMemcpyDeviceToHost));
        const size_t blocks = (size_t)std::min<uint32_t>(handed[0], (uint32_t)cur.motion_ws_layout.queueCap) * 4u, per = 16u * 56u;
        std::vector<uint32_t> dc(blocks * per);
        if (!dc.empty()) LFG_HIP(ctx, hipMemcpy(dc.data(), cur.motion_ws + cur.motion_ws_layout.dynCount, dc.size() * 4, hipMemcpyDeviceToHost));
        size_t hist[40] = {0};
        int dumped = 0;
        const uint32_t deep = (uint32_t)ctx->knobs.debugDynDeep;
        for (size_t i = 0; i < dc.size(); ++i) {
            ++hist[std::min<uint32_t>(dc[i], 39u)];
            if (dc[i] > deep) {
                fprintf(stderr, "lfg: dyn list block %zu (part %zu of its segment) pixel %zu (row %zu, column %zu): %u records\n", i / per, (i / per) % 8u, i % per, (i % per) / 56u, (i % per) % 56u, dc[i]);
                if (dumped++ < 6) {
                    const size_t blk = i / per, row = (i % per) / 56u, col = (i % per) % 56u;
                    const int K = cur.motion_ws_layout.listDyn;
                    for (int k = 0; k < std::min<int>((int)dc[i], K); ++k) {
                        uint32_t rec = 0; float thr = 0.f;
                        (void)hipMemcpy(&rec, cur.motion_ws + cur.motion_ws_layout.dynList + (((blk * 16u + row) * (size_t)K + (size_t)k) * 56u + col) * 4u, 4, hipMemcpyDeviceToHost);
                        (void)hipMemcpy(&thr, cur.motion_ws + cur.motion_ws_layout.dynUmin + ((blk * 16u + row) * 56u + col) * 4u, 4, hipMemcpyDeviceToHost);
                        const uint32_t bits = (rec >> 11) << 10; float c; memcpy(&c, &bits, 4);
                        fprintf(stderr, "      record %2d: cost >= %.3f rank %4u (dx %+d, dy %+d)%s\n", k, c, rec & 0x7FFu, (int)((rec & 0x7FFu) % 33u) - 16, (int)((rec & 0x7FFu) / 33u) - 16, k == 0 ? "" : "");
                        if (k + 1 == std::min<int>((int)dc[i], K)) fprintf(stderr, "      final threshold %.3f\n", thr);
                    }
                }
            }
        }
        {
            const uint32_t ptx = (cur.motion_ws_w + 55u) / 56u, pty = (cur.motion_ws_h + 63u) / 64u;
            std::vector<uint32_t> sm((size_t)ptx * pty * 4u);
            LFG_HIP(ctx, hipMemcpy(sm.data(), cur.motion_ws + cur.motion_ws_layout.segMap, sm.size() * 4, hipMemcpyDeviceToHost));
            for (size_t i = 0; i < flags.size(); ++i) if (flags[i]) {
                const uint32_t fx = (uint32_t)(i % tx), fy = (uint32_t)(i / tx);
                for (uint32_t px = fx * 64u / 56u; px <= std::min(ptx - 1u, (fx * 64u + 63u) / 56u); ++px)
                    for (uint32_t sg = 0; sg < 4u; ++sg)
                        fprintf(stderr, "lfg: flagged tile (%u,%u) flag %#x: prefilter tile (%u,%u) segment %u segMap %#x\n", fx, fy, flags[i], px, fy, sg, sm[((size_t)fy * ptx + px) * 4u + sg]);
            }
        }
        for (size_t b = 0; b < blocks; ++b) {
            bool any = false;
            for (size_t i = 0; i < per && !any; ++i) any = dc[b * per + i] != 0u;
            if (!any) fprintf(stderr, "lfg: dyn block %zu (part %zu) holds no counts\n", b, b % 8u);
        }
        {
            double sum[8] = {0}; size_t n8[8] = {0};
            for (size_t i = 0; i < dc.size(); ++i) { sum[(i / per) % 8u] += dc[i]; ++n8[(i / per) % 8u]; }
            fprintf(stderr, "lfg: mean records per pixel by part:");
            for (int k = 0; k < 8; ++k) fprintf(stderr, " %.2f", n8[k] ? sum[k] / n8[k] : 0.0);
            fprintf(stderr, "\n");
        }
        fprintf(stderr, "lfg: dyn list depths over %zu pixel-parts:", dc.size());
        for (int k = 0; k < 40; ++k) if (hist[k]) fprintf(stderr, " %d:%zu", k, hist[k]);
        fprintf(stderr, "\n");
    }
    if (ctx->knobs.debug)
        for (size_t i = 0; i < flags.size(); ++i)
            if (flags[i]) fprintf(stderr, "lfg: motion fallback tile (%zu, %zu)\n", i % tx, i / tx);
    if (out_tiles) *out_tiles = tx * ty;
    if (out_fallback_tiles) *out_fallback_tiles = fb;
    if (out_mean_recorded) {
        const size_t px = (size_t)cur.motion_ws_w * cur.motion_ws_h;
        std::vector<uint32_t> cnt(px);
        LFG_HIP(ctx, hipMemcpy(cnt.data(), cur.motion_ws + cur.motion_ws_layout.count, px * 4, hipMemcpyDeviceToHost));
        const lfg::PrefilterPlanHost plan = lfg::prefilter_plan(cur.motion_ws_w, cur.motion_ws_h, ctx->motion_slots,
                                                                cur.motion_ws_layout.lastLean ? cur.motion_ws_layout.rimSplit2 : cur.motion_ws_layout.rimSplit);
        std::vector<uint32_t> segDone((size_t)plan.tiles * 4u);
        LFG_HIP(ctx, hipMemcpy(segDone.data(), cur.motion_ws + cur.motion_ws_layout.segDone, segDone.size() * 4, hipMemcpyDeviceToHost));
        double sum = 0; size_t n = 0;
        for (uint32_t y = 0; y < cur.motion_ws_h; ++y)
            for (uint32_t x = 0; x < cur.motion_ws_w; ++x) {
                const size_t ptile = (size_t)(y / 64u) * (size_t)plan.tilesX + x / 56u;
                if (!flags[(size_t)(y / 64u) * tx + x / 64u] && plan.tileMap[ptile] == 0xFFFFFFFFu) {
                    sum += segDone[ptile * 4u + (y % 64u) / 16u] ? 0.0 : (double)cnt[(size_t)y * cur.motion_ws_w + x]; ++n;
                }
            }
        *out_mean_recorded = n ? sum / (double)n : 0.0;
    }
    return LFG_OK;
}

LFG_EXPORT int lfg_interpolate(lfg_context *ctx, const lfg_frame *prev, const lfg_frame *curr, const lfg_frame *mv,
                               lfg_frame *out, float factor) {
    if (!ctx) return LFG_ERR_INVALID;
    LFG_HIP(ctx, hipSetDevice(ctx->device));
    if (!frame_ok(prev, LFG_FORMAT_RGBA8_UNORM) || !frame_ok(curr, LFG_FORMAT_RGBA8_UNORM) ||
        !frame_ok(mv, LFG_FORMAT_MV_S8X2) || !frame_ok(out, LFG_FORMAT_RGBA8_UNORM))
        return fail(ctx, LFG_ERR_INVALID, "lfg_interpolate: bad frame (NULL, empty or wrong format)");
    if (!same_size(prev, curr) || !same_size(curr, mv) || !same_size(curr, out))
        return fail(ctx, LFG_ERR_INVALID, "lfg_interpolate: frames differ in size");
    if ((prev->pitch | curr->pitch | out->pitch) % 4u || mv->pitch % 2u)
        return fail(ctx, LFG_ERR_INVALID, "lfg_interpolate: row pitch not a multiple of the pixel size");
    if (out->data == prev->data || out->data == curr->data)
        return fail(ctx, LFG_ERR_INVALID, "lfg_interpolate: output aliases an input");
    lfg::InterpTables tb;
    int rc = interp_tables(ctx, (int)curr->width, (int)curr->height, &tb);
    if (rc != LFG_OK) return rc;
    StageTimer timer(ctx, LFG_STAGE_INTERPOLATE);
    hipError_t e = lfg::launch_interpolate(ctx->cur().stream, *prev, *curr, *mv, *out, factor, ctx->semantics != 0, tb);
    if (e != hipSuccess) return fail_hip(ctx, e, "interpolate kernel launch");
    return LFG_OK;
}

namespace {

constexpr int kFramesBlockSize = 8;
constexpr float kFramesSearchRadius = 16.0f;

int frame_vectors_into(lfg_context *ctx, const lfg_frame *prev, const lfg_frame *curr, lfg_frame &estimated, lfg_frame &refined,
                       const lfg_frame **vectors) {
    int rc = lane_frame(ctx, estimated, curr->width, curr->height, LFG_FORMAT_MV_S8X2);
    if (rc != LFG_OK) return fail(ctx, rc, "Failed to create motion vectors frame");
    if (ctx->half_res_radius >= 0) {
        lfg_lane_state &cur = ctx->cur();
        const uint32_t hw = (curr->width + 1u) / 2u, hh = (curr->height + 1u) / 2u;
        rc = lane_frame(ctx, cur.half_prev, hw, hh, LFG_FORMAT_RGBA8_UNORM);
        if (rc == LFG_OK) rc = lane_frame(ctx, cur.half_curr, hw, hh, LFG_FORMAT_RGBA8_UNORM);
        if (rc == LFG_OK) rc = lane_frame(ctx, cur.mv_half, hw, hh, LFG_FORMAT_MV_S8X2);
        if (rc != LFG_OK) return fail(ctx, rc, "Failed to create the half-resolution motion frames");
        if (!frame_ok(prev, LFG_FORMAT_RGBA8_UNORM) || !frame_ok(curr, LFG_FORMAT_RGBA8_UNORM) || !same_size(prev, curr))
            return fail(ctx, LFG_ERR_INVALID, "lfg_interpolate_frames: prev and curr must be non-empty RGBA8 frames of one size");
        rc = lfg_frame_halve(ctx, prev, &cur.half_prev);
        if (rc == LFG_OK) rc = lfg_frame_halve(ctx, curr, &cur.half_curr);
        if (rc == LFG_OK)
            rc = ctx->estimator == LFG_ESTIMATOR_PYRAMID
                     ? lfg_motion_pyramid(ctx, &cur.half_prev, &cur.half_curr, &cur.mv_half, 1, 16, 2)
                     : lfg_motion(ctx, &cur.half_prev, &cur.half_curr, &cur.mv_half, kFramesBlockSize, kFramesSearchRadius);
        if (rc == LFG_OK) rc = lfg_motion_expand(ctx, prev, curr, &cur.mv_half, &estimated, ctx->half_res_radius);
    } else {
        rc = ctx->estimator == LFG_ESTIMATOR_PYRAMID ? lfg_motion_pyramid(ctx, prev, curr, &estimated, 2, 16, 2)
                                                     : lfg_motion(ctx, prev, curr, &estimated, kFramesBlockSize, kFramesSearchRadius);
    }
    if (rc != LFG_OK) return rc;
    *vectors = &estimated;
    if (ctx->refine_radius < 0) return LFG_OK;
    rc = lane_frame(ctx, refined, curr->width, curr->height, LFG_FORMAT_MV_S8X2);
    if (rc != LFG_OK) return fail(ctx, rc, "Failed to create refined motion vectors frame");
    *vectors = &refined;
    return lfg_motion_refine(ctx, prev, curr, &estimated, &refined, ctx->refine_radius);
}

int frame_vectors(lfg_context *ctx, const lfg_frame *prev, const lfg_frame *curr, const lfg_frame **vectors) {
    lfg_lane_state &cur = ctx->cur();
    return frame_vectors_into(ctx, prev, curr, cur.mv_tmp, cur.mv_refined, vectors);
}

bool bidirectional_applies(const lfg_context *ctx) {
    return ctx->bidir_tolerance >= 0 && ctx->interpolator == LFG_INTERPOLATOR_COMPENSATED &&
           ctx->generation == LFG_GENERATION_INTERPOLATE && ctx->static_tolerance < 0;
}

int cut_fallback_check(lfg_context *ctx, const lfg_frame *prev, const lfg_frame *curr, const void *device_stats,
                       int min_matched_permille, lfg_frame *const *outs, const float *factors, uint32_t count);
int compensated_frames(lfg_context *ctx, const lfg_frame *prev, const lfg_frame *curr, const lfg_frame *vectors,
                       lfg_frame *const *outs, const float *factors, uint32_t count, bool multi);
int cut_fallback_enqueue(lfg_context *ctx, const lfg_frame *prev, const lfg_frame *curr, const void *device_stats,
                         int min_matched_permille, lfg_frame *const *outs, const float *factors, uint32_t count);

int detecting_frames(lfg_context *ctx, const lfg_frame *prev, const lfg_frame *curr, lfg_frame *const *outs, const float *factors,
                     uint32_t count, bool multi) {
    LFG_HIP(ctx, hipSetDevice(ctx->device));
    lfg::CutDetectState &cut = ctx->cur().cut;
    if (!cut.device) LFG_HIP(ctx, hipMalloc((void **)&cut.device, sizeof(lfg_pair_stats)));
    if (!cut.pinned) LFG_HIP(ctx, hipHostMalloc((void **)&cut.pinned, sizeof(lfg_pair_stats), hipHostMallocDefault));
    if (!cut.event) LFG_HIP(ctx, hipEventCreateWithFlags(&cut.event, hipEventDisableTiming));
    const int permille = ctx->cut_permille;
    int rc = cut_fallback_check(ctx, prev, curr, cut.device, permille, outs, factors, count);
    if (rc != LFG_OK) return rc;
    const lfg_frame *vectors = nullptr;
    rc = frame_vectors(ctx, prev, curr, &vectors);
    if (rc != LFG_OK) return rc;
    rc = lfg_pair_match(ctx, prev, curr, vectors, ctx->match_sad, cut.device);
    if (rc != LFG_OK) return rc;
    LFG_HIP(ctx, hipMemcpyAsync(cut.pinned, cut.device, sizeof(lfg_pair_stats), hipMemcpyDeviceToHost, ctx->cur().stream));
    LFG_HIP(ctx, hipEventRecord(cut.event, ctx->cur().stream));
    cut.recorded = true;
    cut.permille = permille;
    if (ctx->interpolator == LFG_INTERPOLATOR_COMPENSATED)
        rc = compensated_frames(ctx, prev, curr, vectors, outs, factors, count, multi);
    else
        rc = multi ? lfg_interpolate_multi(ctx, prev, curr, vectors, outs, factors, count)
                   : lfg_interpolate(ctx, prev, curr, vectors, outs[0], factors[0]);
    if (rc != LFG_OK) return rc;
    if (ctx->generation == LFG_GENERATION_EXTRAPOLATE && ctx->interpolator == LFG_INTERPOLATOR_COMPENSATED) {
        float newest[LFG_MAX_FACTORS];
        for (uint32_t i = 0; i < count; ++i) newest[i] = 1.0f;
        return cut_fallback_enqueue(ctx, prev, curr, cut.device, permille, outs, newest, count);
    }
    return cut_fallback_enqueue(ctx, prev, curr, cut.device, permille, outs, factors, count);
}

}

LFG_EXPORT int lfg_interpolate_frames(lfg_context *ctx, const lfg_frame *prev, const lfg_frame *curr,
                                      lfg_frame *out, float factor) {
    if (!ctx || !curr) return fail(ctx, LFG_ERR_INVALID, "lfg_interpolate_frames: NULL argument");
    if (ctx->cut_permille >= 0) {
        lfg_frame *const outs[1] = {out};
        return detecting_frames(ctx, prev, curr, outs, &factor, 1, false);
    }
    if (ctx->fuse_motion_interpolate && ctx->estimator == LFG_ESTIMATOR_FULL_SEARCH && ctx->refine_radius < 0 &&
        ctx->half_res_radius < 0 && ctx->interpolator == LFG_INTERPOLATOR_SHADER) {
        lfg_frame &mv = ctx->cur().mv_tmp;
        int rc = lane_frame(ctx, mv, curr->width, curr->height, LFG_FORMAT_MV_S8X2);
        if (rc != LFG_OK) return fail(ctx, rc, "Failed to create motion vectors frame");
        if (!frame_ok(prev, LFG_FORMAT_RGBA8_UNORM) || !frame_ok(out, LFG_FORMAT_RGBA8_UNORM) || !same_size(curr, out) || out->pitch % 4u)
            return fail(ctx, LFG_ERR_INVALID, "lfg_interpolate_frames: bad output frame (NULL, empty, wrong format, size or pitch)");
        if (out->data == prev->data || out->data == curr->data)
            return fail(ctx, LFG_ERR_INVALID, "lfg_interpolate_frames: the output aliases an input");
        lfg::FusedOut fo;
        fo.data = (uint8_t *)out->data; fo.pitch = (int)out->pitch; fo.t = factor; fo.intended = ctx->semantics != 0 ? 1 : 0; fo.storeMv = 0;
        bool done = false;
        rc = motion_run(ctx, prev, curr, &mv, kFramesBlockSize, kFramesSearchRadius, &fo, &done);
        if (rc != LFG_OK || done) return rc;
        return lfg_interpolate(ctx, prev, curr, &mv, out, factor);
    }
    const lfg_frame *vectors = nullptr;
    int rc = frame_vectors(ctx, prev, curr, &vectors);
    if (rc != LFG_OK) return rc;
    if (ctx->interpolator == LFG_INTERPOLATOR_COMPENSATED) {
        lfg_frame *const outs[1] = {out};
        return compensated_frames(ctx, prev, curr, vectors, outs, &factor, 1, false);
    }
    return lfg_interpolate(ctx, prev, curr, vectors, out, factor);
}

LFG_EXPORT int lfg_interpolate_multi(lfg_context *ctx, const lfg_frame *prev, const lfg_frame *curr, const lfg_frame *mv,
                                     lfg_frame *const *outs, const float *factors, uint32_t count) {
    if (!ctx) return LFG_ERR_INVALID;
    LFG_HIP(ctx, hipSetDevice(ctx->device));
    if (!outs || !factors || count == 0 || count > LFG_MAX_FACTORS)
        return fail(ctx, LFG_ERR_INVALID, "lfg_interpolate_multi: count must be in [1, LFG_MAX_FACTORS] and outs/factors non-NULL");
    if (!frame_ok(prev, LFG_FORMAT_RGBA8_UNORM) || !frame_ok(curr, LFG_FORMAT_RGBA8_UNORM) || !frame_ok(mv, LFG_FORMAT_MV_S8X2))
        return fail(ctx, LFG_ERR_INVALID, "lfg_interpolate_multi: bad frame (NULL, empty or wrong format)");
    if (!same_size(prev, curr) || !same_size(curr, mv))
        return fail(ctx, LFG_ERR_INVALID, "lfg_interpolate_multi: frames differ in size");
    if ((prev->pitch | curr->pitch) % 4u || mv->pitch % 2u)
        return fail(ctx, LFG_ERR_INVALID, "lfg_interpolate_multi: row pitch not a multiple of the pixel size");
    for (uint32_t i = 0; i < count; ++i) {
        const lfg_frame *o = outs[i];
        if (!frame_ok(o, LFG_FORMAT_RGBA8_UNORM) || !same_size(curr, o) || o->pitch % 4u)
            return fail(ctx, LFG_ERR_INVALID, "lfg_interpolate_multi: bad output frame (NULL, empty, wrong format, size or pitch)");
        if (o->data == prev->data || o->data == curr->data)
            return fail(ctx, LFG_ERR_INVALID, "lfg_interpolate_multi: an output aliases an input");
        for (uint32_t j = 0; j < i; ++j)
            if (outs[j]->data == o->data) return fail(ctx, LFG_ERR_INVALID, "lfg_interpolate_multi: two outputs alias each other");
    }
    lfg::InterpTables tb;
    int rc = interp_tables(ctx, (int)curr->width, (int)curr->height, &tb);
    if (rc != LFG_OK) return rc;
    StageTimer timer(ctx, LFG_STAGE_INTERPOLATE);
    hipError_t e = lfg::launch_interpolate_multi(ctx->cur().stream, *prev, *curr, *mv, outs, factors, (int)count, ctx->semantics != 0, tb);
    if (e != hipSuccess) return fail_hip(ctx, e, "interpolate kernel launch");
    return LFG_OK;
}

LFG_EXPORT int lfg_interpolate_frames_multi(lfg_context *ctx, const lfg_frame *prev, const lfg_frame *curr,
                                            lfg_frame *const *outs, const float *factors, uint32_t count) {
    if (!ctx || !curr) return fail(ctx, LFG_ERR_INVALID, "lfg_interpolate_frames_multi: NULL argument");
    if (ctx->cut_permille >= 0) return detecting_frames(ctx, prev, curr, outs, factors, count, true);
    const lfg_frame *vectors = nullptr;
    int rc = frame_vectors(ctx, prev, curr, &vectors);
    if (rc != LFG_OK) return rc;
    if (ctx->interpolator == LFG_INTERPOLATOR_COMPENSATED) return compensated_frames(ctx, prev, curr, vectors, outs, factors, count, true);
    return lfg_interpolate_multi(ctx, prev, curr, vectors, outs, factors, count);
}


namespace {

bool frames_overlap(const lfg_frame *a, const lfg_frame *b) {
    const uintptr_t a0 = (uintptr_t)a->data, b0 = (uintptr_t)b->data;
    const uintptr_t a1 = a0 + (size_t)a->pitch * (a->height - 1u) + (size_t)a->width * bytes_per_pixel(a->format);
    const uintptr_t b1 = b0 + (size_t)b->pitch * (b->height - 1u) + (size_t)b->width * bytes_per_pixel(b->format);
    return a0 < b1 && b0 < a1;
}

bool mask_overlaps(const lfg_mask *m, const lfg_frame *f) {
    const uintptr_t a0 = (uintptr_t)m->data, b0 = (uintptr_t)f->data;
    const uintptr_t a1 = a0 + (size_t)m->pitch * (m->height - 1u) + (size_t)m->width;
    const uintptr_t b1 = b0 + (size_t)f->pitch * (f->height - 1u) + (size_t)f->width * bytes_per_pixel(f->format);
    return a0 < b1 && b0 < a1;
}

bool mask_ok(const lfg_mask *m, const lfg_frame *like) {
    return m && m->data && m->width == like->width && m->height == like->height && m->pitch >= m->width;
}

enum class McKind { Plain, Masked, Extrapolate, Bidirectional, Subpel };

int compensated_run(lfg_context *ctx, const lfg_frame *prev, const lfg_frame *curr, const lfg_frame *mv, const lfg_mask *mask, McKind kind,
                    lfg_frame *const *outs, const float *factors, uint32_t count, int match_sad, const char *name,
                    const lfg_frame *bwd = nullptr, int tolerance = 0) {
    const bool masked = kind == McKind::Masked, bidir = kind == McKind::Bidirectional, subpel = kind == McKind::Subpel;
    const uint32_t mvFormat = subpel ? LFG_FORMAT_MV_S16X2_Q2 : LFG_FORMAT_MV_S8X2, mvAlign = subpel ? 4u : 2u;
    if (!ctx) return LFG_ERR_INVALID;
    LFG_HIP(ctx, hipSetDevice(ctx->device));
    const std::string n(name);
    if (!outs || !factors || count == 0 || count > LFG_MAX_FACTORS)
        return fail(ctx, LFG_ERR_INVALID, n + ": count must be in [1, LFG_MAX_FACTORS] and outs/factors non-NULL");
    if (!frame_ok(prev, LFG_FORMAT_RGBA8_UNORM) || !frame_ok(curr, LFG_FORMAT_RGBA8_UNORM) || !frame_ok(mv, mvFormat))
        return fail(ctx, LFG_ERR_INVALID, n + (subpel ? ": prev/curr must be RGBA8 and mvq MV_S16X2_Q2, all non-empty"
                                                      : ": prev/curr must be RGBA8 and mv MV_S8X2, all non-empty"));
    if (!same_size(prev, curr) || !same_size(curr, mv))
        return fail(ctx, LFG_ERR_INVALID, n + ": prev, curr and mv differ in size");
    if ((prev->pitch | curr->pitch) % 4u || ((uintptr_t)prev->data | (uintptr_t)curr->data) % 4u || mv->pitch % mvAlign || (uintptr_t)mv->data % mvAlign)
        return fail(ctx, LFG_ERR_INVALID, n + (subpel ? ": RGBA8 frames and mvq must be 4-byte aligned"
                                                      : ": RGBA8 frames must be 4-byte aligned and mv 2-byte aligned"));
    if (match_sad < 0 || match_sad > 1020) return fail(ctx, LFG_ERR_INVALID, n + ": match_sad must be in [0, 1020]");
    if (masked && !mask_ok(mask, curr))
        return fail(ctx, LFG_ERR_INVALID, n + ": mask must be non-NULL, of the frames' size, with pitch >= width");
    if (bidir && (!frame_ok(bwd, LFG_FORMAT_MV_S8X2) || !same_size(curr, bwd) || bwd->pitch % 2u || (uintptr_t)bwd->data % 2u))
        return fail(ctx, LFG_ERR_INVALID, n + ": bwd must be a non-empty, 2-byte aligned MV_S8X2 frame of the frames' size");
    if (bidir && (tolerance < 0 || tolerance > 64)) return fail(ctx, LFG_ERR_INVALID, n + ": tolerance must be in [0, 64]");
    for (uint32_t i = 0; i < count; ++i) {
        const lfg_frame *o = outs[i];
        if (!frame_ok(o, LFG_FORMAT_RGBA8_UNORM) || !same_size(curr, o) || o->pitch % 4u || (uintptr_t)o->data % 4u)
            return fail(ctx, LFG_ERR_INVALID, n + ": bad output frame (NULL, empty, wrong format, size or alignment)");
        if (!std::isfinite(factors[i]) || factors[i] < 0.0f || factors[i] > 1.0f)
            return fail(ctx, LFG_ERR_INVALID, n + ": every factor must be a finite number in [0, 1]");
        if (frames_overlap(o, prev) || frames_overlap(o, curr) || frames_overlap(o, mv) || (masked && mask_overlaps(mask, o)) ||
            (bidir && frames_overlap(o, bwd)))
            return fail(ctx, LFG_ERR_INVALID, n + ": an output aliases an input");
        for (uint32_t j = 0; j < i; ++j)
            if (frames_overlap(outs[j], o)) return fail(ctx, LFG_ERR_INVALID, n + ": two outputs alias each other");
    }
    lfg_lane_state &cur = ctx->cur();
    const size_t bytes = (size_t)curr->width * curr->height * 4u;
    int rc = subpel ? lane_buffer_grow(ctx, cur.mcq_keys, cur.mcq_keys_bytes, 2u * bytes, "hipMalloc((void **)&cur.mcq_keys, 2 * bytes)")
                    : lane_buffer_grow(ctx, cur.mc_keys, cur.mc_keys_bytes, bytes, "hipMalloc((void **)&cur.mc_keys, bytes)");
    if (rc != LFG_OK) return rc;
    const int reach = kind == McKind::Extrapolate || subpel ? -1 : ctx->hole_reach;
    if (reach >= 1) {
        rc = lane_buffer_grow(ctx, cur.mc_fill, cur.mc_fill_bytes, bytes, "hipMalloc((void **)&cur.mc_fill, bytes)");
        if (rc != LFG_OK) return rc;
    }
    uint32_t *const fill = reach >= 1 ? cur.mc_fill : nullptr;
    StageTimer timer(ctx, LFG_STAGE_INTERPOLATE);
    for (uint32_t i = 0; i < count; ++i) {
        hipError_t e = subpel ? lfg::launch_interpolate_compensated_subpel(cur.stream, *prev, *curr, *mv, *outs[i], factors[i], match_sad, cur.mcq_keys)
                       : masked ? lfg::launch_interpolate_compensated_masked(cur.stream, *prev, *curr, *mv, *mask, *outs[i], factors[i], match_sad, cur.mc_keys,
                                                                           fill, reach)
                       : kind == McKind::Extrapolate
                              ? lfg::launch_extrapolate_compensated(cur.stream, *prev, *curr, *mv, *outs[i], factors[i], match_sad, cur.mc_keys)
                       : bidir ? lfg::launch_interpolate_compensated_bidirectional(cur.stream, *prev, *curr, *mv, *bwd, *outs[i], factors[i],
                                                                                   match_sad, tolerance, cur.mc_keys, fill, reach)
                              : lfg::launch_interpolate_compensated(cur.stream, *prev, *curr, *mv, *outs[i], factors[i], match_sad, cur.mc_keys,
                                                                    fill, reach);
        if (e != hipSuccess) return fail_hip(ctx, e, kind == McKind::Extrapolate ? "compensated extrapolate kernel launch" : "compensated interpolate kernel launch");
    }
    return LFG_OK;
}

bool subpixel_applies(const lfg_context *ctx) {
    return ctx->subpel_radius >= 0 && ctx->interpolator == LFG_INTERPOLATOR_COMPENSATED && ctx->generation == LFG_GENERATION_INTERPOLATE &&
           ctx->bidir_tolerance < 0 && ctx->static_tolerance < 0 && ctx->hole_reach < 0;
}

int compensated_frames(lfg_context *ctx, const lfg_frame *prev, const lfg_frame *curr, const lfg_frame *vectors,
                       lfg_frame *const *outs, const float *factors, uint32_t count, bool multi) {
    if (ctx->generation == LFG_GENERATION_EXTRAPOLATE)
        return compensated_run(ctx, prev, curr, vectors, nullptr, McKind::Extrapolate, outs, factors, count, ctx->match_sad,
                               multi ? "lfg_extrapolate_compensated_multi" : "lfg_extrapolate_compensated");
    if (bidirectional_applies(ctx)) {
        lfg_lane_state &cur = ctx->cur();
        const lfg_frame *backward = nullptr;
        const int rc = frame_vectors_into(ctx, curr, prev, cur.mv_bwd, cur.mv_bwd_refined, &backward);
        if (rc != LFG_OK) return rc;
        return compensated_run(ctx, prev, curr, vectors, nullptr, McKind::Bidirectional, outs, factors, count, ctx->match_sad,
                               multi ? "lfg_interpolate_compensated_bidirectional_multi" : "lfg_interpolate_compensated_bidirectional",
                               backward, ctx->bidir_tolerance);
    }
    if (subpixel_applies(ctx)) {
        lfg_lane_state &cur = ctx->cur();
        int rc = lane_frame(ctx, cur.mvq_tmp, curr->width, curr->height, LFG_FORMAT_MV_S16X2_Q2);
        if (rc != LFG_OK) return fail(ctx, rc, "Failed to create the quarter-pixel motion vectors frame");
        rc = lfg_motion_subpel(ctx, prev, curr, vectors, &cur.mvq_tmp, ctx->subpel_radius);
        if (rc != LFG_OK) return rc;
        return compensated_run(ctx, prev, curr, &cur.mvq_tmp, nullptr, McKind::Subpel, outs, factors, count, ctx->match_sad,
                               multi ? "lfg_interpolate_compensated_subpel_multi" : "lfg_interpolate_compensated_subpel");
    }
    if (ctx->static_tolerance < 0)
        return compensated_run(ctx, prev, curr, vectors, nullptr, McKind::Plain, outs, factors, count, ctx->match_sad,
                               multi ? "lfg_interpolate_compensated_multi" : "lfg_interpolate_compensated");
    LFG_HIP(ctx, hipSetDevice(ctx->device));
    lfg_lane_state &cur = ctx->cur();
    const size_t bytes = (size_t)curr->width * curr->height;
    int rc = lane_buffer_grow(ctx, cur.static_mask, cur.static_mask_bytes, bytes, "hipMalloc((void **)&cur.static_mask, bytes)");
    if (rc != LFG_OK) return rc;
    const lfg_mask mask{cur.static_mask, curr->width, curr->height, curr->width};
    rc = lfg_static_mask(ctx, prev, curr, ctx->static_tolerance, &mask);
    if (rc != LFG_OK) return rc;
    return compensated_run(ctx, prev, curr, vectors, &mask, McKind::Masked, outs, factors, count, ctx->match_sad,
                           multi ? "lfg_interpolate_compensated_masked_multi" : "lfg_interpolate_compensated_masked");
}

}

LFG_EXPORT int lfg_interpolate_compensated(lfg_context *ctx, const lfg_frame *prev, const lfg_frame *curr, const lfg_frame *mv,
                                           lfg_frame *out, float factor, int match_sad) {
    lfg_frame *const outs[1] = {out};
    return compensated_run(ctx, prev, curr, mv, nullptr, McKind::Plain, outs, &factor, 1, match_sad, "lfg_interpolate_compensated");
}

LFG_EXPORT int lfg_interpolate_compensated_multi(lfg_context *ctx, const lfg_frame *prev, const lfg_frame *curr, const lfg_frame *mv,
                                                 lfg_frame *const *outs, const float *factors, uint32_t count, int match_sad) {
    return compensated_run(ctx, prev, curr, mv, nullptr, McKind::Plain, outs, factors, count, match_sad, "lfg_interpolate_compensated_multi");
// ... 751 lines not shown
```

### linux-fg_amd/csrc/lfg_internal.hpp

```cpp
#pragma once

#include <hip/hip_runtime.h>

#include <cstdint>
#include <string>
#include <vector>

#include "linuxfg_hip.h"
#include "lfg_motion_verdict.hpp"
#include "lfg_resample.hpp"

namespace lfg {

struct AxisTable {
    int in_size = 0, out_size = 0;
    bool pattern_2x = false;
    int *d_start = nullptr;
    float *d_weight = nullptr;
    uint8_t *d_class = nullptr;
    float *d_palette = nullptr;
    int palette_rows = 0;
    int strips_per_xcd = 0;
};

struct UvTable {
    int size = 0;
    float *d_uv = nullptr;
    uint8_t *d_centre = nullptr;
    uint64_t *d_goodMask = nullptr;
    int blocks = 0;
    float rcp = 0.0f;
    bool rcpExact = false;
};

struct InterpTables {
    const float *uvx = nullptr, *uvy = nullptr;
    const uint8_t *centreX = nullptr, *centreY = nullptr;
    const uint64_t *goodMask = nullptr;
    float rcpW = 0.0f, rcpH = 0.0f;
    int rcpExact = 0;
};

struct FusedOut {
    uint8_t *data = nullptr;
    int pitch = 0;
    float t = 0.5f;
    int intended = 0;
    int storeMv = 1;
};

enum MotionCtrlWord : int {
    kCtrlNextUnit = 0,
    kCtrlUnitsDone = 1,
    kCtrlNextSlot = 2,
    kCtrlOpenCount = 4,
    kCtrlHardCount = 5,
    kCtrlLeanSettled = 6,
    kCtrlLeanLeft = 7,
};

struct MotionWorkspaceLayout { size_t colBand, rowBand ; size_t verdict , orderFlags; size_t list, umin, count, tileFlags, segDone, segMap, queueCount, ctrl, order, plan, auxList, auxUmin, auxCount,
                               queue, dynList, dynUmin, dynCount, dynInit, openList, merge, mergeBytes, leanTiles, hardTiles, plan2, total; int queueCap, slots, rimSplit, listMain, listAux, listDyn, leanCount, leanLaunch , rimSplit2, units, units2, units2Static , tiles, lastLean ; };
struct PrefilterPlan {
    int tilesX, units;
    const uint32_t *unitMap;
    const uint32_t *unitAux;
    const uint32_t *tileMap;
    uint32_t *auxList;
    float *auxUmin;
    uint32_t *auxCount;
    uint32_t *segMap;
    uint32_t *queueCount;
    uint32_t *queue;
    int queueCap;
    uint32_t *dynList;
    float *dynUmin;
    uint32_t *dynCount;
    uint32_t *dynInit;
    int dynParts;
    uint32_t *openList, *openCount;
    const uint32_t *colBand, *rowBand;
    int unitsStatic;
    const uint32_t *hardTiles, *hardCount;
    FusedOut fused;
};
struct PrefilterPlanHost {
    int tilesX = 0, tiles = 0, units = 0, auxUnits = 0;
    std::vector<uint32_t> unitMap, unitAux, tileMap;
    std::vector<uint32_t> leanTiles;
    std::vector<uint32_t> leanPartial;
};

constexpr int kPyramidMaxLevels = 4;
struct PyramidLayout {
    int levels = 0;
    uint32_t w[kPyramidMaxLevels + 1] = {}, h[kPyramidMaxLevels + 1] = {};
    size_t prev[kPyramidMaxLevels + 1] = {}, curr[kPyramidMaxLevels + 1] = {}, mv[kPyramidMaxLevels + 1] = {};
    size_t total = 0;
};

struct ResampleTable {
    int filter = 0;
    uint32_t in_size = 0, out_size = 0;
    uint8_t *d_base = nullptr;
    ResampleAxis axis{};
    ResamplePlan plan{};
};

struct ProfileSlot {
    hipEvent_t begin = nullptr, end = nullptr;
    int stage = 0;
};

struct CutDetectState {
    lfg_pair_stats *device = nullptr;
    lfg_pair_stats *pinned = nullptr;
    hipEvent_t event = nullptr;
    bool recorded = false;
    int permille = -1;
};

}

struct lfg_lane_state {
    hipStream_t own_stream = nullptr, stream = nullptr;
    lfg_frame mv_tmp{};
    lfg_frame mv_refined{};
    lfg_frame mv_bwd{}, mv_bwd_refined{};
    lfg_frame half_prev{}, half_curr{}, mv_half{};
    lfg_frame mid_tmp{};
    uint8_t *motion_ws = nullptr;
    size_t motion_ws_bytes = 0;
    uint32_t motion_ws_w = 0, motion_ws_h = 0;
    lfg::MotionWorkspaceLayout motion_ws_layout{};
    int motion_units = 0;
    uint8_t *pyramid_ws = nullptr;
    size_t pyramid_ws_bytes = 0;
    uint32_t *mc_keys = nullptr;
    size_t mc_keys_bytes = 0;
    uint32_t *mc_fill = nullptr;
    size_t mc_fill_bytes = 0;
    uint8_t *static_mask = nullptr;
    size_t static_mask_bytes = 0;
    lfg_frame mvq_tmp{};
    unsigned long long *mcq_keys = nullptr;
    size_t mcq_keys_bytes = 0;
    hipEvent_t mark = nullptr;
    bool marked = false;
    lfg::MotionVerdictState verdict;
    lfg::CutDetectState cut;
};

struct lfg_context {
    int device = 0;
    int device_cus = 0;
    std::vector<lfg_lane_state> lanes;
    int lane = 0;
    lfg_lane_state &cur() { return lanes[(size_t)lane]; }
    const lfg_lane_state &cur() const { return lanes[(size_t)lane]; }
    lfg_lane_state &from_selected(size_t k) { return lanes[((size_t)lane + k) % lanes.size()]; }
    uint64_t pred_verdicts = 0, pred_lean_wrong = 0, pred_grid_wrong = 0, pred_second_wrong = 0;
    std::string error;
    std::vector<lfg::AxisTable> tables;
    std::vector<lfg::UvTable> uv_tables;
    std::vector<lfg::ResampleTable> resample_tables;
    int motion_slots = 0;
    int rim_split_env = 0;
    int motion_mode = 0;
    int semantics = 0;
    int estimator = 0;
    int interpolator = 0;
    int match_sad = 48;
    int refine_radius = -1;
    int cut_permille = -1;
    int static_tolerance = -1;
    int generation = 0;
    int bidir_tolerance = -1;
    int hole_reach = -1;
    int half_res_radius = -1;
    int subpel_radius = -1;
    uint32_t *motion_tables = nullptr;
    bool fuse_interpolate_scale = false;
    bool fuse_motion_interpolate = false;
    bool motion_hints = true;
    bool motion_lean = true;
    lfg::MotionKnobs knobs;
    void *comm = nullptr;
    int comm_ranks = 0, comm_rank = 0;
    hipStream_t comm_stream = nullptr;
    hipEvent_t comm_ready = nullptr, comm_done = nullptr;
    bool comm_pending = false;
    hipEvent_t probe_begin = nullptr, probe_end = nullptr;
    int scale_last_kernel = -1;
    int motion_last_tier = 0;
    int comm_cus = 0;
    bool profile = false;
    std::vector<lfg::ProfileSlot> prof_pending;
    std::vector<std::pair<hipEvent_t, hipEvent_t>> prof_free;
    double prof_ms[LFG_STAGE_COUNT] = {0, 0, 0};
    uint64_t prof_n[LFG_STAGE_COUNT] = {0, 0, 0};
};

hipError_t lfg_own_stream_create(const lfg_context *ctx, hipStream_t *out);
int lfg_restream(lfg_context *ctx);

namespace lfg {

hipError_t launch_comm_probe(hipStream_t s, int workgroups, int microseconds);

hipError_t launch_scale_generic(hipStream_t s, const lfg_frame &in, const lfg_frame &out,
                                const AxisTable &tx, const AxisTable &ty);
hipError_t launch_scale_2x(hipStream_t s, const lfg_frame &in, const lfg_frame &out,
                           const AxisTable &tx, const AxisTable &ty);
bool scale_2x_supported(const lfg_frame &in, const lfg_frame &out);
hipError_t launch_interpolate_scale_2x(hipStream_t s, const lfg_frame &prev, const lfg_frame &curr, const lfg_frame &mv,
                                       const lfg_frame &out, const AxisTable &tx, const AxisTable &ty, float factor, bool intended);
int scale_2x_strips_per_xcd(int inH);
void scale_2x_strip_host(int inH, int xcd, int index, int &first, int &steps);
hipError_t launch_motion_tiled_8_16(hipStream_t s, const lfg_frame &prev, const lfg_frame &curr,
                                    const lfg_frame &mv, const uint32_t *tileFlags, const uint32_t *rank2scan,
                                    unsigned long long *merge = nullptr, uint32_t *flaggedTiles = nullptr, const FusedOut &fused = FusedOut(),
                                    bool expectNothing = false, uint32_t *verdictWord = nullptr, uint32_t *hostWord = nullptr);
constexpr int kMotionTableWords = 1092;
void motion_tables(bool intended, uint32_t *rank2scan, uint32_t *order32, uint32_t *entryOfScan, uint32_t *baseScan);
size_t motion_workspace_bytes(uint32_t width, uint32_t height, int slots, int rimSplit, int rimSplit2, MotionWorkspaceLayout *layout);
PrefilterPlanHost prefilter_plan(uint32_t width, uint32_t height, int slots, int rimSplit);
int prefilter_slots();
hipError_t launch_motion_prefiltered_8_16(hipStream_t s, const lfg_frame &prev, const lfg_frame &curr,
                                          const lfg_frame &mv, uint8_t *workspace, const MotionWorkspaceLayout &layout, int units,
                                          const uint32_t *rank2scan, const uint32_t *order32,
                                          const uint32_t *entryOfScan, const uint32_t *baseScan, bool useHints, bool framesInFlight,
                                          const FusedOut &fused = FusedOut(), bool lean = false, uint32_t *leanFlagHost = nullptr,
                                          int groupsCap = 0 ,
                                          bool expectNoFallback = false ,
                                          const MotionKnobs &knobs = MotionKnobs(), bool rankIsScan = true,
                                          int tier = 0 );
hipError_t launch_motion_order(hipStream_t s, const lfg_frame &prev, const lfg_frame &curr, uint32_t *hints, uint32_t *callOrder,
                               const uint32_t *entryOfScan, const uint32_t *baseScan, uint32_t *clearFrom, int clearWords, bool framesInFlight);
hipError_t launch_motion_resolve(hipStream_t s, const lfg_frame &prev, const lfg_frame &curr, const lfg_frame &mv, const uint32_t *list,
                                 const float *umin, const uint32_t *count, const uint32_t *tileFlags, int tilesX, const PrefilterPlan &sp,
                                 const uint32_t *rank2scan, const uint32_t *segDone, int groups);
bool lean_tile_ok(int tile, int tilesX, int W, int H);
bool lean_segment_ok(int tile, int seg, int tilesX, int W, int H);
bool lean_frames_ok(const lfg_frame &prev, const lfg_frame &curr, const lfg_frame &mv);
hipError_t launch_motion_lean(hipStream_t s, const lfg_frame &prev, const lfg_frame &curr, const lfg_frame &mv,
                              const uint32_t *order32, const uint32_t *rank2scan, bool rankIsScan ,
                              const uint32_t *leanTiles, int nTiles, int tilesX, uint32_t *segDone,
                              uint32_t *hardTiles, uint32_t *hardCount, uint32_t *stats, bool whateverTheVerdict);
bool strip_frames_ok(const lfg_frame &prev, const lfg_frame &curr, const lfg_frame &mv);
hipError_t launch_motion_strip(hipStream_t s, const lfg_frame &prev, const lfg_frame &curr, const lfg_frame &mv, const uint32_t *order32,
                               const uint32_t *rank2scan, bool rankIsScan, uint32_t *colBand, uint32_t *rowBand,
                               uint32_t *tileFlags, uint32_t *flagged, int flagTilesX, int ldsPad);
hipError_t launch_motion_generic(hipStream_t s, const lfg_frame &prev, const lfg_frame &curr,
                                 const lfg_frame &mv, int block_size, int radius, bool intended);
hipError_t launch_interpolate(hipStream_t s, const lfg_frame &prev, const lfg_frame &curr,
                              const lfg_frame &mv, const lfg_frame &out, float factor, bool intended, const InterpTables &tb);
hipError_t launch_interpolate_multi(hipStream_t s, const lfg_frame &prev, const lfg_frame &curr, const lfg_frame &mv,
                                    const lfg_frame *const *outs, const float *factors, int count, bool intended,
                                    const InterpTables &tb);
size_t pyramid_workspace_bytes(uint32_t width, uint32_t height, int levels, PyramidLayout *layout);
hipError_t launch_motion_pyramid(hipStream_t s, const lfg_frame &prev, const lfg_frame &curr, const lfg_frame &mv,
                                 int levels, int coarseRadius, int refineRadius, uint8_t *workspace, const PyramidLayout &layout);
hipError_t launch_hole_fill_plane(hipStream_t s, const uint32_t *keys, size_t keysPitchWords, uint32_t *plane, size_t planePitchWords,
                                  int W, int H, int reach, bool passStatic, int band = 0);
hipError_t launch_interpolate_compensated(hipStream_t s, const lfg_frame &prev, const lfg_frame &curr, const lfg_frame &mv,
                                          const lfg_frame &out, float factor, int matchSad, uint32_t *keys, uint32_t *fill = nullptr,
                                          int reach = 0);
hipError_t launch_interpolate_compensated_masked(hipStream_t s, const lfg_frame &prev, const lfg_frame &curr, const lfg_frame &mv,
                                                 const lfg_mask &mask, const lfg_frame &out, float factor, int matchSad, uint32_t *keys,
                                                 uint32_t *fill = nullptr, int reach = 0);
hipError_t launch_static_mask(hipStream_t s, const lfg_frame &prev, const lfg_frame &curr, int tolerance, const lfg_mask &out);
hipError_t launch_extrapolate_compensated(hipStream_t s, const lfg_frame &prev, const lfg_frame &curr, const lfg_frame &mv,
                                          const lfg_frame &out, float ahead, int matchSad, uint32_t *keys);
hipError_t launch_interpolate_compensated_bidirectional(hipStream_t s, const lfg_frame &prev, const lfg_frame &curr, const lfg_frame &fwd,
                                                        const lfg_frame &bwd, const lfg_frame &out, float factor, int matchSad,
                                                        int tolerance, uint32_t *keys, uint32_t *fill = nullptr, int reach = 0);
hipError_t launch_motion_consistency(hipStream_t s, const lfg_frame &a, const lfg_frame &b, int tolerance, const lfg_mask &out);
hipError_t launch_motion_refine(hipStream_t s, const lfg_frame &prev, const lfg_frame &curr, const lfg_frame &mvIn,
                                const lfg_frame &mvOut, int radius);
hipError_t launch_frame_halve(hipStream_t s, const lfg_frame &in, const lfg_frame &out);
hipError_t launch_motion_expand(hipStream_t s, const lfg_frame &prev, const lfg_frame &curr, const lfg_frame &mvLow,
                                const lfg_frame &mvOut, int radius);
hipError_t launch_motion_subpel(hipStream_t s, const lfg_frame &prev, const lfg_frame &curr, const lfg_frame &mvIn,
                                const lfg_frame &mvqOut, int radius);
hipError_t launch_interpolate_compensated_subpel(hipStream_t s, const lfg_frame &prev, const lfg_frame &curr, const lfg_frame &mvq,
                                                 const lfg_frame &out, float factor, int matchSad, unsigned long long *keys);
hipError_t launch_pair_match(hipStream_t s, const lfg_frame &prev, const lfg_frame &curr, const lfg_frame &mv, int matchSad,
                             int deviceCus, void *stats);
hipError_t launch_cut_fallback(hipStream_t s, const lfg_frame &prev, const lfg_frame &curr, const void *stats, int minMatchedPermille,
                               const lfg_frame *const *outs, const float *factors, int count, int deviceCus);
hipError_t launch_frame_diff(hipStream_t s, const lfg_frame &a, const lfg_frame &b, uint32_t channelMask, bool accumulate,
                             int deviceCus, void *stats);
struct YuvCoefficients { int32_t to_rgb[5]; int32_t to_yuv[9]; int32_t offset; };
bool yuv_grid_ok(uint32_t width, uint32_t height);
hipError_t launch_nv12_to_rgba(hipStream_t s, const lfg_nv12 &in, const lfg_frame &out, const YuvCoefficients &k, int siting);
hipError_t launch_rgba_to_nv12(hipStream_t s, const lfg_frame &in, const lfg_nv12 &out, const YuvCoefficients &k, int siting);
hipError_t launch_sharpen(hipStream_t s, const lfg_frame &in, const lfg_frame &out, int strength);
hipError_t launch_resample(hipStream_t s, const lfg_frame &in, const lfg_frame &out, const ResampleAxis &x, const ResampleAxis &y,
                           const ResamplePlan &plan);
hipError_t launch_mv_export(hipStream_t s, const lfg_frame &mv, float *rgba32f);
hipError_t launch_sqrt_selftest(hipStream_t s, uint32_t lo_bits, uint32_t hi_bits, unsigned long long *d_mismatch);

}
```

Before: 3935 frames/s.

## Route interpolation through reject-and-compact pass when most pixels fall out of range

Adds a reject kernel that zero-fills 8-pixel groups whose motion vectors push both taps out of range. It appends the remaining groups to a compacted list, which a persistent list kernel then interpolates. The default interpolate kernel now samples per-tile how many pixels could be in range and reports the counts to pinned host memory through an event. The host uses these counts to pick the reject route on later calls. This adds sampling overhead, an extra launch, and host-side state in exchange for skipping work on frames dominated by large motion.

```diff
diff --git a/include/linuxfg_hip.h b/include/linuxfg_hip.h
--- a/include/linuxfg_hip.h
+++ b/include/linuxfg_hip.h
@@ -101,6 +101,7 @@
 int  lfg_motion_lean_stats(lfg_context *ctx, int *out_used, uint32_t *out_tiles, uint32_t *out_tiles_left);
 int  lfg_motion_strip_stats(lfg_context *ctx, uint32_t *out_rows, uint32_t *out_columns);
 int  lfg_motion_last_variant(const lfg_context *ctx);
+int  lfg_interpolate_last_route(const lfg_context *ctx);
 int  lfg_motion_prediction_stats(const lfg_context *ctx, uint64_t *out_verdicts, uint64_t *out_lean_wrong,
                                  uint64_t *out_grid_wrong, uint64_t *out_second_pass_wrong);
 int  lfg_motion_workspace_size(lfg_context *ctx, uint32_t width, uint32_t height, uint64_t *out_bytes);
diff --git a/linux-fg_amd/capi.py b/linux-fg_amd/capi.py
--- a/linux-fg_amd/capi.py
+++ b/linux-fg_amd/capi.py
@@ -183,6 +183,7 @@
     "lfg_broadcast_frame_lane": (_i, [_vp, _FP, _i]),
     "lfg_comm_probe_ms": (_i, [_vp, ctypes.POINTER(ctypes.c_float)]),
     "lfg_motion_last_variant": (_i, [_vp]),
+    "lfg_interpolate_last_route": (_i, [_vp]),
     "lfg_scale_last_kernel": (_i, [_vp]),
     "lfg_diag_scale_2x_strip": (_i, [_u32, _u32, _u32, ctypes.POINTER(_u32), ctypes.POINTER(ctypes.c_int32), ctypes.POINTER(ctypes.c_int32)]),
     "lfg_profile_enable": (_i, [_vp, _i]),
@@ -429,6 +430,9 @@
     def motion_last_variant(self) -> int:
         return int(self.lib.lfg_motion_last_variant(self.h))
 
+    def interpolate_last_route(self) -> int:
+        return int(self.lib.lfg_interpolate_last_route(self.h))
+
     def motion_plan(self):
         a, b = ctypes.c_int(), ctypes.c_int()
         self._check(self.lib.lfg_motion_plan(self.h, ctypes.byref(a), ctypes.byref(b)), "lfg_motion_plan")
diff --git a/linux-fg_amd/csrc/interpolate.hip b/linux-fg_amd/csrc/interpolate.hip
--- a/linux-fg_amd/csrc/interpolate.hip
+++ b/linux-fg_amd/csrc/interpolate.hip
@@ -109,15 +109,28 @@
 };
 
 template <int N, bool INTENDED>
-__global__ __launch_bounds__(256, N == 1 ? LFG_INTERP_WAVES : LFG_INTERP_WAVES_MULTI) void interpolate_kernel(
+__device__ __forceinline__ void generic_pixel(const uint8_t *__restrict__ prev, int prevPitch, const uint8_t *__restrict__ curr, int currPitch,
+                                              int W, int H, int8_t mx, int8_t my, float uvx, float uvy, const MultiTargets &tg, uint32_t *o, const int stride) {
+    const bool still = mx == 0 && my == 0;
+    SampleTaps sp, sc;
+    SampleTexels tp, tc;
+#pragma unroll
+    for (int k = 0; k < N; ++k) {
+        const float t = tg.t[k];
+        if (k == 0 || !still) {
+            o[k * stride] = 0u;
+            if (!pixel_taps<INTENDED>(prev, prevPitch, curr, currPitch, W, H, mx, my, uvx, uvy, t, sp, sc)) continue;
+            tp = sample_load(sp); tc = sample_load(sc);
+        }
+        o[k * stride] = pixel_finish(sp, tp, sc, tc, t);
+    }
+}
+
+template <int N, bool INTENDED>
+__device__ __forceinline__ void interpolate_quad(
     const uint8_t *__restrict__ prev, int prevPitch, const uint8_t *__restrict__ curr, int currPitch,
-    const int8_t *__restrict__ mv, int mvPitch, MultiTargets tg, int W, int H, bool wideStores,
-    InterpTables tb, int fast) {
-    const int lane = threadIdx.x & 63;
-    const int py = blockIdx.y * 4 + (threadIdx.x >> 6);
-    if (py >= H) return;
-    const int px0 = (blockIdx.x * 64 + lane) * 4;
-    if (px0 >= W) return;
+    const int8_t *__restrict__ mv, int mvPitch, const MultiTargets &tg, int W, int H, bool wideStores,
+    const InterpTables &tb, int fast, const int px0, const int py, const int maskWord, const int maskBit) {
 #ifdef LFG_DIAG_INTERP_ROWS_CENTRE
     const bool rowCentre = fast;
 #else
@@ -144,7 +157,7 @@
 #ifdef LFG_DIAG_INTERP_NO_PATCH
             const bool laneGood = true;
 #else
-            const bool laneGood = ((tb.goodMask[blockIdx.x] >> lane) & 1ull) != 0ull;
+            const bool laneGood = ((tb.goodMask[maskWord] >> maskBit) & 1ull) != 0ull;
 #endif
             V4 fp[4], fc[4];
             if (laneGood) {
@@ -170,7 +183,7 @@
             return;
         }
         if (fast && zero) {
-            const bool laneGood = ((tb.goodMask[blockIdx.x] >> lane) & 1ull) != 0ull;
+            const bool laneGood = ((tb.goodMask[maskWord] >> maskBit) & 1ull) != 0ull;
             const RowTaps ty = row_taps(py, H, uv_div(py, H));
             const int j0 = ty.below ? py - 1 : py;
             const int r0 = clampi(j0, 0, H - 1), r1 = clampi(j0 + 1, 0, H - 1);
@@ -248,19 +261,7 @@
     for (int i = 0; i < 4; ++i) uvxOf[i] = uv_of(min(px0 + i, W - 1), W, tb.rcpW, tb.rcpExact, tb.uvx);
 #pragma unroll
     for (int i = 0; i < 4; ++i) {
-        const bool still = m[2 * i] == 0 && m[2 * i + 1] == 0;
-        SampleTaps sp, sc;
-        SampleTexels tp, tc;
-#pragma unroll
-        for (int k = 0; k < N; ++k) {
-            const float t = tg.t[k];
-            if (k == 0 || !still) {
-                o[k][i] = 0u;
-                if (!pixel_taps<INTENDED>(prev, prevPitch, curr, currPitch, W, H, m[2 * i], m[2 * i + 1], uvxOf[i], uvy, t, sp, sc)) continue;
-                tp = sample_load(sp); tc = sample_load(sc);
-            }
-            o[k][i] = pixel_finish(sp, tp, sc, tc, t);
-        }
+        generic_pixel<N, INTENDED>(prev, prevPitch, curr, currPitch, W, H, m[2 * i], m[2 * i + 1], uvxOf[i], uvy, tg, &o[0][i], 4);
     }
 #pragma unroll
     for (int k = 0; k < N; ++k) {
@@ -274,25 +275,202 @@
     }
 }
 
+struct InterpSample {
+    uint32_t *words = nullptr;
+    int rowShift = 0, minOut = 0;
+};
+
+template <int N, bool INTENDED, bool SAMPLE>
+__global__ __launch_bounds__(256, N == 1 ? LFG_INTERP_WAVES : LFG_INTERP_WAVES_MULTI) void interpolate_kernel(
+    const uint8_t *__restrict__ prev, int prevPitch, const uint8_t *__restrict__ curr, int currPitch,
+    const int8_t *__restrict__ mv, int mvPitch, MultiTargets tg, int W, int H, bool wideStores,
+    InterpTables tb, int fast, InterpSample sample) {
+    const int lane = threadIdx.x & 63;
+    const int py = blockIdx.y * 4 + (threadIdx.x >> 6);
+    if (py >= H) return;
+    const int px0 = (blockIdx.x * 64 + lane) * 4;
+    if (SAMPLE && threadIdx.x < 64 && (blockIdx.y & ((1u << sample.rowShift) - 1u)) == 0u) {
+        bool may = false;
+        if (px0 < W) {
+#pragma unroll
+            for (int i = 0; i < 4; ++i) {
+                const int8_t *m = mv + (size_t)py * (size_t)mvPitch + (size_t)min(px0 + i, W - 1) * 2u;
+                may = may || max(abs((int)m[0]), abs((int)m[1])) < sample.minOut;
+            }
+        }
+        const unsigned long long mayMask = __ballot(may), quadMask = __ballot(px0 < W);
+        if (lane == 0)
+            __hip_atomic_store(&sample.words[(blockIdx.y >> sample.rowShift) * gridDim.x + blockIdx.x],
+                               (uint32_t)__builtin_popcountll(mayMask) | ((uint32_t)__builtin_popcountll(quadMask) << 16), __ATOMIC_RELAXED, __HIP_MEMORY_SCOPE_SYSTEM);
+    }
+    if (px0 >= W) return;
+    interpolate_quad<N, INTENDED>(prev, prevPitch, curr, currPitch, mv, mvPitch, tg, W, H, wideStores, tb, fast, px0, py, (int)blockIdx.x, lane);
+}
+
+#ifndef LFG_INTERP_REJECT_ROWS
+#define LFG_INTERP_REJECT_ROWS 8
+#endif
+constexpr int kRejectRows = LFG_INTERP_REJECT_ROWS;
+constexpr int kListGroups = 512;
+
+template <int N>
+__global__ __launch_bounds__(256) void interpolate_reject_kernel(const int8_t *__restrict__ mv, int mvPitch, MultiTargets tg, int groupsPerRow, int H,
+                                                                 uint32_t *__restrict__ list, uint32_t *__restrict__ count, uint32_t listCap) {
+    const int lane = threadIdx.x & 63;
+    const int g = blockIdx.x * 64 + lane;
+    const int row0 = (blockIdx.y * 4 + (threadIdx.x >> 6)) * kRejectRows;
+    if (row0 >= H) return;
+    const bool mine = g < groupsPerRow;
+    const int gc = mine ? g : groupsPerRow - 1;
+    uint4 mm[kRejectRows];
+    uint32_t listedRows = 0u;
+#pragma unroll
+    for (int r = 0; r < kRejectRows; ++r)
+        mm[r] = *reinterpret_cast<const uint4 *>(mv + (size_t)min(row0 + r, H - 1) * (size_t)mvPitch + (size_t)gc * 16u);
+#pragma unroll
+    for (int r = 0; r < kRejectRows; ++r) {
+        const int py = row0 + r;
+        if (py >= H) break;
+        const uint32_t w[4] = {mm[r].x, mm[r].y, mm[r].z, mm[r].w};
+        bool allOut = true;
+#pragma unroll
+        for (int k = 0; k < N; ++k) {
+            const float t = tg.t[k], sa = -t, sb = 1.0f - t;
+#pragma unroll
+            for (int i = 0; i < 8; ++i) {
+                const uint32_t two = w[i >> 1] >> (16 * (i & 1));
+                const float mx = (float)(int8_t)(two & 0xffu), my = (float)(int8_t)((two >> 8) & 0xffu);
+                const bool outA = __builtin_fabsf(mx * sa) >= 1.0f || __builtin_fabsf(my * sa) >= 1.0f;
+                const bool outB = __builtin_fabsf(mx * sb) >= 1.0f || __builtin_fabsf(my * sb) >= 1.0f;
+                allOut = allOut && outA && outB;
+            }
+        }
+        if (mine && allOut) {
+#pragma unroll
+            for (int k = 0; k < N; ++k) {
+                uint8_t *o = tg.out[k] + (size_t)py * (size_t)tg.pitch[k] + (size_t)g * 32u;
+                *reinterpret_cast<uint4 *>(o) = uint4{0u, 0u, 0u, 0u};
+                *reinterpret_cast<uint4 *>(o + 16) = uint4{0u, 0u, 0u, 0u};
+            }
+        }
+        listedRows |= (mine && !allOut) ? 1u << r : 0u;
+    }
+    uint32_t total = 0u;
+#pragma unroll
+    for (int r = 0; r < kRejectRows; ++r) total += (uint32_t)__builtin_popcountll(__ballot(((listedRows >> r) & 1u) != 0u));
+    if (total == 0u) return;
+    uint32_t base = 0u;
+    if (lane == 0) base = atomicAdd(count, total);
+    base = (uint32_t)__builtin_amdgcn_readfirstlane((int)base);
+#pragma unroll
+    for (int r = 0; r < kRejectRows; ++r) {
+        const bool listed = ((listedRows >> r) & 1u) != 0u;
+        const unsigned long long b = __ballot(listed);
+        const uint32_t at = base + (uint32_t)__builtin_popcountll(b & ((1ull << lane) - 1ull));
+        if (listed && at < listCap) list[at] = (uint32_t)((row0 + r) * groupsPerRow + g);
+        base += (uint32_t)__builtin_popcountll(b);
+    }
+}
+
+template <int N>
+__global__ __launch_bounds__(256) void interpolate_list_kernel(
+    const uint8_t *__restrict__ prev, int prevPitch, const uint8_t *__restrict__ curr, int currPitch,
+    const int8_t *__restrict__ mv, int mvPitch, MultiTargets tg, int W, int H, InterpTables tb,
+    const uint32_t *__restrict__ list, const uint32_t *__restrict__ countWord, uint32_t *__restrict__ nextCount, uint32_t *__restrict__ hostWord, int groupsPerRow) {
+    const uint32_t count = min(*countWord, (uint32_t)(groupsPerRow * H));
+    if (blockIdx.x == 0 && threadIdx.x == 0) {
+        *nextCount = 0u;
+        if (hostWord) __hip_atomic_store(hostWord, count, __ATOMIC_RELAXED, __HIP_MEMORY_SCOPE_SYSTEM);
+    }
+    const int lane = threadIdx.x & 63;
+    const uint32_t waves = gridDim.x * 4u;
+    for (uint32_t c = blockIdx.x * 4u + (threadIdx.x >> 6); c * 8u < count; c += waves) {
+        const uint32_t at = c * 8u + (uint32_t)(lane >> 3);
+        if (at < count) {
+            const uint32_t group = list[at];
+            const int py = (int)(group / (uint32_t)groupsPerRow);
+            const int px = ((int)group - py * groupsPerRow) * 8 + (lane & 7);
+            const int8_t *m = mv + (size_t)py * (size_t)mvPitch + (size_t)px * 2u;
+            uint32_t o[N];
+            generic_pixel<N, false>(prev, prevPitch, curr, currPitch, W, H, m[0], m[1], uv_of(px, W, tb.rcpW, tb.rcpExact, tb.uvx),
+                                    uv_of(py, H, tb.rcpH, tb.rcpExact, tb.uvy), tg, o, 1);
+#pragma unroll
+            for (int k = 0; k < N; ++k) *reinterpret_cast<uint32_t *>(tg.out[k] + (size_t)py * (size_t)tg.pitch[k] + (size_t)px * 4u) = o[k];
+        }
+    }
+}
+
 template <int N>
 static void launch_n(hipStream_t s, dim3 grid, const lfg_frame &prev, const lfg_frame &curr, const lfg_frame &mv,
-                     const MultiTargets &tg, int W, int H, bool wide, bool intended, const InterpTables &tb, int fast) {
+                     const MultiTargets &tg, int W, int H, bool wide, bool intended, const InterpTables &tb, int fast, const InterpSample &sample) {
     if (intended)
-        hipLaunchKernelGGL((interpolate_kernel<N, true>), grid, dim3(256), 0, s,
+        hipLaunchKernelGGL((interpolate_kernel<N, true, false>), grid, dim3(256), 0, s,
                            (const uint8_t *)prev.data, (int)prev.pitch, (const uint8_t *)curr.data, (int)curr.pitch,
-                           (const int8_t *)mv.data, (int)mv.pitch, tg, W, H, wide, tb, fast);
+                           (const int8_t *)mv.data, (int)mv.pitch, tg, W, H, wide, tb, fast, InterpSample());
+    else if (sample.words)
+        hipLaunchKernelGGL((interpolate_kernel<N, false, true>), grid, dim3(256), 0, s,
+                           (const uint8_t *)prev.data, (int)prev.pitch, (const uint8_t *)curr.data, (int)curr.pitch,
+                           (const int8_t *)mv.data, (int)mv.pitch, tg, W, H, wide, tb, fast, sample);
     else
-        hipLaunchKernelGGL((interpolate_kernel<N, false>), grid, dim3(256), 0, s,
+        hipLaunchKernelGGL((interpolate_kernel<N, false, false>), grid, dim3(256), 0, s,
                            (const uint8_t *)prev.data, (int)prev.pitch, (const uint8_t *)curr.data, (int)curr.pitch,
-                           (const int8_t *)mv.data, (int)mv.pitch, tg, W, H, wide, tb, fast);
+                           (const int8_t *)mv.data, (int)mv.pitch, tg, W, H, wide, tb, fast, InterpSample());
+}
+
+template <int N>
+static void launch_reject_n(hipStream_t s, const lfg_frame &prev, const lfg_frame &curr, const lfg_frame &mv, const MultiTargets &tg,
+                            int W, int H, const InterpTables &tb, InterpRoute &route) {
+    const int groupsPerRow = W / 8;
+    uint32_t *const count = route.ctrl + (route.turn & 1), *const nextCount = route.ctrl + ((route.turn + 1) & 1);
+    route.turn = (route.turn + 1) & 1;
+    hipLaunchKernelGGL((interpolate_reject_kernel<N>), dim3((groupsPerRow + 63) / 64, (H + 4 * kRejectRows - 1) / (4 * kRejectRows)), dim3(256), 0, s,
+                       (const int8_t *)mv.data, (int)mv.pitch, tg, groupsPerRow, H, route.list, count, (uint32_t)(groupsPerRow * H));
+    hipLaunchKernelGGL((interpolate_list_kernel<N>), dim3(kListGroups), dim3(256), 0, s,
+                       (const uint8_t *)prev.data, (int)prev.pitch, (const uint8_t *)curr.data, (int)curr.pitch,
+                       (const int8_t *)mv.data, (int)mv.pitch, tg, W, H, tb, route.list, count, nextCount, route.host, groupsPerRow);
+}
+
+bool interpolate_reject_ok(const lfg_frame &prev, const lfg_frame &curr, const lfg_frame &mv, const lfg_frame *const *outs, int count,
+                           bool intended, const InterpTables &tb) {
+    if (intended || curr.width % 8u != 0u || !fast_frames(prev, curr, mv) || !tb.goodMask || curr.width >= (1u << 20) || curr.height >= (1u << 20)) return false;
+    if (mv.pitch % 16u != 0u || (uintptr_t)mv.data % 16u != 0u) return false;
+    for (int i = 0; i < count; ++i)
+        if (!fast_output(*outs[i]) || (uint64_t)outs[i]->pitch * outs[i]->height >= (1ull << 31)) return false;
+    return true;
 }
 
 hipError_t launch_interpolate_multi(hipStream_t s, const lfg_frame &prev, const lfg_frame &curr, const lfg_frame &mv,
                                     const lfg_frame *const *outs, const float *factors, int count, bool intended,
-                                    const InterpTables &tb) {
+                                    const InterpTables &tb, InterpRoute *route) {
     const int W = (int)curr.width, H = (int)curr.height;
     const int quads = (W + 3) / 4;
     const dim3 grid((quads + 63) / 64, (H + 3) / 4);
+    if (route && route->reject) {
+        for (int first = 0; first < count; first += kMaxMulti) {
+            const int n = count - first < kMaxMulti ? count - first : kMaxMulti;
+            MultiTargets tg{};
+            for (int k = 0; k < kMaxMulti; ++k) {
+                const lfg_frame &o = *outs[first + (k < n ? k : 0)];
+                tg.out[k] = (uint8_t *)o.data; tg.pitch[k] = (int)o.pitch; tg.t[k] = factors[first + (k < n ? k : 0)];
+            }
+            switch (n) {
+                case 1: launch_reject_n<1>(s, prev, curr, mv, tg, W, H, tb, *route); break;
+                case 2: launch_reject_n<2>(s, prev, curr, mv, tg, W, H, tb, *route); break;
+                case 3: launch_reject_n<3>(s, prev, curr, mv, tg, W, H, tb, *route); break;
+                default: launch_reject_n<4>(s, prev, curr, mv, tg, W, H, tb, *route); break;
+            }
+            hipError_t e = hipGetLastError();
+            if (e != hipSuccess) return e;
+        }
+        return hipSuccess;
+    }
+    InterpSample sample;
+    if (route && route->host && !intended) {
+        while ((int)grid.x * (((int)grid.y + (1 << sample.rowShift) - 1) >> sample.rowShift) > kInterpSampleWords && sample.rowShift < 30) ++sample.rowShift;
+        sample.words = route->host + 1;
+        route->sampleWords = (int)grid.x * (((int)grid.y + (1 << sample.rowShift) - 1) >> sample.rowShift);
+        if (route->sampleWords > kInterpSampleWords) { sample.words = nullptr; route->sampleWords = 0; }
+    }
     for (int first = 0; first < count; first += kMaxMulti) {
         const int n = count - first < kMaxMulti ? count - first : kMaxMulti;
         MultiTargets tg{};
@@ -303,11 +481,18 @@
             wide = wide && fast_output(o);
         }
         const int fast = fast_frames(prev, curr, mv) && wide && tb.goodMask && W < (1 << 20) && H < (1 << 20) ? 1 : 0;
+        sample.minOut = 129;
+        for (int m = 128; m >= 1; --m) {
+            bool out = true;
+            for (int k = 0; k < n; ++k) out = out && __builtin_fabsf((float)m * -tg.t[k]) >= 1.0f && __builtin_fabsf((float)m * (1.0f - tg.t[k])) >= 1.0f;
+            if (!out) break;
+            sample.minOut = m;
+        }
         switch (n) {
-            case 1: launch_n<1>(s, grid, prev, curr, mv, tg, W, H, wide, intended, tb, fast); break;
-            case 2: launch_n<2>(s, grid, prev, curr, mv, tg, W, H, wide, intended, tb, fast); break;
-            case 3: launch_n<3>(s, grid, prev, curr, mv, tg, W, H, wide, intended, tb, fast); break;
-            default: launch_n<4>(s, grid, prev, curr, mv, tg, W, H, wide, intended, tb, fast); break;
+            case 1: launch_n<1>(s, grid, prev, curr, mv, tg, W, H, wide, intended, tb, fast, sample); break;
+            case 2: launch_n<2>(s, grid, prev, curr, mv, tg, W, H, wide, intended, tb, fast, sample); break;
+            case 3: launch_n<3>(s, grid, prev, curr, mv, tg, W, H, wide, intended, tb, fast, sample); break;
+            default: launch_n<4>(s, grid, prev, curr, mv, tg, W, H, wide, intended, tb, fast, sample); break;
         }
         hipError_t e = hipGetLastError();
         if (e != hipSuccess) return e;
@@ -316,9 +501,9 @@
 }
 
 hipError_t launch_interpolate(hipStream_t s, const lfg_frame &prev, const lfg_frame &curr,
-                              const lfg_frame &mv, const lfg_frame &out, float factor, bool intended, const InterpTables &tb) {
+                              const lfg_frame &mv, const lfg_frame &out, float factor, bool intended, const InterpTables &tb, InterpRoute *route) {
     const lfg_frame *outs[1] = {&out};
-    return launch_interpolate_multi(s, prev, curr, mv, outs, &factor, 1, intended, tb);
+    return launch_interpolate_multi(s, prev, curr, mv, outs, &factor, 1, intended, tb, route);
 }
 
 __global__ __launch_bounds__(256) void mv_export_kernel(const int8_t *__restrict__ mv, int mvPitch,
diff --git a/linux-fg_amd/csrc/lfg_capi.cpp b/linux-fg_amd/csrc/lfg_capi.cpp
--- a/linux-fg_amd/csrc/lfg_capi.cpp
+++ b/linux-fg_amd/csrc/lfg_capi.cpp
@@ -405,6 +405,7 @@
     ctx->tables.reserve(17);
     if (const char *m = getenv("LFG_MOTION_HINTS")) ctx->motion_hints = atoi(m) != 0;
     if (const char *m = getenv("LFG_MOTION_LEAN")) ctx->motion_lean = atoi(m) != 0;
+    if (const char *m = getenv("LFG_INTERP_REJECT")) ctx->interp_reject = atoi(m) != 0;
     if (const char *m = getenv("LFG_MOTION_RIM_SPLIT")) { const int v = atoi(m); if (v == 4 || v == 8 || v == 48) ctx->rim_split_env = v; }
     if (const char *m = getenv("LFG_FUSED_INTERPOLATE_SCALE")) ctx->fuse_interpolate_scale = atoi(m) != 0;
     if (const char *m = getenv("LFG_FUSED_MOTION_INTERPOLATE")) ctx->fuse_motion_interpolate = atoi(m) != 0;
@@ -444,6 +445,10 @@
     if (l.cut.event) (void)hipEventDestroy(l.cut.event);
     if (l.cut.pinned) (void)hipHostFree(l.cut.pinned);
     if (l.cut.device) (void)hipFree(l.cut.device);
+    if (l.reject.event) (void)hipEventDestroy(l.reject.event);
+    if (l.reject.pinned) (void)hipHostFree(l.reject.pinned);
+    if (l.reject.ctrl) (void)hipFree(l.reject.ctrl);
+    if (l.reject.list) (void)hipFree(l.reject.list);
     if (l.own_stream) (void)hipStreamDestroy(l.own_stream);
     l = lfg_lane_state{};
 }
@@ -1024,6 +1029,66 @@
     return LFG_OK;
 }
 
+namespace {
+
+int interp_route_begin(lfg_context *ctx, const lfg_frame &prev, const lfg_frame &curr, const lfg_frame &mv, const lfg_frame *const *outs,
+                       int count, const lfg::InterpTables &tb, lfg::InterpRoute *route) {
+    *route = lfg::InterpRoute();
+    ctx->cur().interp_last_route = 0;
+    if (ctx->interp_reject == 0 || !lfg::interpolate_reject_ok(prev, curr, mv, outs, count, ctx->semantics != 0, tb)) return LFG_OK;
+    lfg_lane_state &cur = ctx->cur();
+    lfg::InterpRejectState &r = cur.reject;
+    if (!r.ready) {
+        if (!r.pinned) LFG_HIP(ctx, hipHostMalloc((void **)&r.pinned, (1 + lfg::kInterpSampleWords) * sizeof(uint32_t), hipHostMallocDefault));
+        memset(r.pinned, 0, (1 + lfg::kInterpSampleWords) * sizeof(uint32_t));
+        if (!r.event) LFG_HIP(ctx, hipEventCreateWithFlags(&r.event, hipEventDisableTiming));
+        if (!r.ctrl) LFG_HIP(ctx, hipMalloc((void **)&r.ctrl, 2 * sizeof(uint32_t)));
+        LFG_HIP(ctx, hipMemsetAsync(r.ctrl, 0, 2 * sizeof(uint32_t), cur.stream));
+        r.turn = 0;
+        r.ready = true;
+    }
+    const size_t groups = (size_t)(curr.width / 8u) * curr.height;
+    if (groups > r.listWords) {
+        LFG_HIP(ctx, hipStreamSynchronize(cur.stream));
+        if (r.list) (void)hipFree(r.list);
+        r.list = nullptr; r.listWords = 0;
+        LFG_HIP(ctx, hipMalloc((void **)&r.list, groups * sizeof(uint32_t)));
+        r.listWords = groups;
+    }
+    if (r.pending && hipEventQuery(r.event) == hipSuccess) {
+        uint64_t may = 0, all = 0;
+        if (r.pendingReject) { may = r.pinned[0]; all = r.groups; }
+        else for (int i = 0; i < r.sampleWords; ++i) { may += r.pinned[1 + i] & 0xFFFFu; all += r.pinned[1 + i] >> 16; }
+        r.busy = all == 0 || may * (uint64_t)lfg::kInterpBusyOneIn > all;
+        r.known = true; r.pending = false;
+    }
+    route->list = r.list; route->ctrl = r.ctrl; route->turn = r.turn;
+    route->reject = ctx->interp_reject == 1 || (ctx->interp_reject < 0 && r.known && !r.busy);
+    cur.interp_last_route = route->reject ? 1 : 0;
+    const bool report = route->reject || (ctx->interp_reject < 0 && ((!r.known && !r.pending) || ++r.unsampled >= lfg::kInterpSampleEvery));
+    if (report) { route->host = r.pinned; r.unsampled = 0; }
+    return LFG_OK;
+}
+
+void interp_route_failed(lfg_context *ctx, const lfg::InterpRoute &route) {
+    if (route.ctrl) ctx->cur().reject.turn = route.turn;
+}
+
+int interp_route_end(lfg_context *ctx, const lfg_frame &curr, const lfg::InterpRoute &route) {
+    lfg_lane_state &cur = ctx->cur();
+    lfg::InterpRejectState &r = cur.reject;
+    if (route.ctrl) r.turn = route.turn;
+    if (!route.host) return LFG_OK;
+    r.pendingReject = route.reject; r.sampleWords = route.sampleWords; r.groups = (uint32_t)((size_t)(curr.width / 8u) * curr.height);
+    LFG_HIP(ctx, hipEventRecord(r.event, cur.stream));
+    r.pending = true;
+    return LFG_OK;
+}
+
+}
+
+LFG_EXPORT int lfg_interpolate_last_route(const lfg_context *ctx) { return ctx ? ctx->lanes[(size_t)ctx->lane].interp_last_route : -1; }
+
 LFG_EXPORT int lfg_interpolate(lfg_context *ctx, const lfg_frame *prev, const lfg_frame *curr, const lfg_frame *mv,
                                lfg_frame *out, float factor) {
     if (!ctx) return LFG_ERR_INVALID;
@@ -1040,10 +1105,14 @@
     lfg::InterpTables tb;
     int rc = interp_tables(ctx, (int)curr->width, (int)curr->height, &tb);
     if (rc != LFG_OK) return rc;
+    lfg::InterpRoute route;
+    const lfg_frame *outs[1] = {out};
+    rc = interp_route_begin(ctx, *prev, *curr, *mv, outs, 1, tb, &route);
+    if (rc != LFG_OK) return rc;
     StageTimer timer(ctx, LFG_STAGE_INTERPOLATE);
-    hipError_t e = lfg::launch_interpolate(ctx->cur().stream, *prev, *curr, *mv, *out, factor, ctx->semantics != 0, tb);
-    if (e != hipSuccess) return fail_hip(ctx, e, "interpolate kernel launch");
-    return LFG_OK;
+    hipError_t e = lfg::launch_interpolate(ctx->cur().stream, *prev, *curr, *mv, *out, factor, ctx->semantics != 0, tb, &route);
+    if (e != hipSuccess) { interp_route_failed(ctx, route); return fail_hip(ctx, e, "interpolate kernel launch"); }
+    return interp_route_end(ctx, *curr, route);
 }
 
 namespace {
@@ -1193,10 +1262,13 @@
     lfg::InterpTables tb;
     int rc = interp_tables(ctx, (int)curr->width, (int)curr->height, &tb);
     if (rc != LFG_OK) return rc;
+    lfg::InterpRoute route;
+    rc = interp_route_begin(ctx, *prev, *curr, *mv, outs, (int)count, tb, &route);
+    if (rc != LFG_OK) return rc;
     StageTimer timer(ctx, LFG_STAGE_INTERPOLATE);
-    hipError_t e = lfg::launch_interpolate_multi(ctx->cur().stream, *prev, *curr, *mv, outs, factors, (int)count, ctx->semantics != 0, tb);
-    if (e != hipSuccess) return fail_hip(ctx, e, "interpolate kernel launch");
-    return LFG_OK;
+    hipError_t e = lfg::launch_interpolate_multi(ctx->cur().stream, *prev, *curr, *mv, outs, factors, (int)count, ctx->semantics != 0, tb, &route);
+    if (e != hipSuccess) { interp_route_failed(ctx, route); return fail_hip(ctx, e, "interpolate kernel launch"); }
+    return interp_route_end(ctx, *curr, route);
 }
 
 LFG_EXPORT int lfg_interpolate_frames_multi(lfg_context *ctx, const lfg_frame *prev, const lfg_frame *curr,
diff --git a/linux-fg_amd/csrc/lfg_internal.hpp b/linux-fg_amd/csrc/lfg_internal.hpp
--- a/linux-fg_amd/csrc/lfg_internal.hpp
+++ b/linux-fg_amd/csrc/lfg_internal.hpp
@@ -39,6 +39,34 @@
     const uint64_t *goodMask = nullptr;
     float rcpW = 0.0f, rcpH = 0.0f;
     int rcpExact = 0;
+};
+
+constexpr int kInterpSampleWords = 256;
+constexpr int kInterpSampleEvery = 16;
+constexpr int kInterpBusyOneIn = 8;
+struct InterpRoute {
+    bool reject = false;
+    uint32_t *list = nullptr;
+    uint32_t *ctrl = nullptr;
+    int turn = 0;
+    uint32_t *host = nullptr;
+    int sampleWords = 0;
+};
+
+struct InterpRejectState {
+    uint32_t *list = nullptr;
+    size_t listWords = 0;
+    uint32_t *ctrl = nullptr;
+    uint32_t *pinned = nullptr;
+    hipEvent_t event = nullptr;
+    bool ready = false;
+    bool pending = false;
+    bool pendingReject = false;
+    int sampleWords = 0;
+    uint32_t groups = 0;
+    bool known = false, busy = true;
+    int turn = 0;
+    int unsampled = 0;
 };
 
 struct FusedOut {
@@ -149,6 +177,8 @@
     bool marked = false;
     lfg::MotionVerdictState verdict;
     lfg::CutDetectState cut;
+    int interp_last_route = 0;
+    lfg::InterpRejectState reject;
 };
 
 struct lfg_context {
@@ -184,6 +214,7 @@
     bool fuse_motion_interpolate = false;
     bool motion_hints = true;
     bool motion_lean = true;
+    int interp_reject = -1;
     lfg::MotionKnobs knobs;
     void *comm = nullptr;
     int comm_ranks = 0, comm_rank = 0;
@@ -254,10 +285,12 @@
 hipError_t launch_motion_generic(hipStream_t s, const lfg_frame &prev, const lfg_frame &curr,
                                  const lfg_frame &mv, int block_size, int radius, bool intended);
 hipError_t launch_interpolate(hipStream_t s, const lfg_frame &prev, const lfg_frame &curr,
-                              const lfg_frame &mv, const lfg_frame &out, float factor, bool intended, const InterpTables &tb);
+                              const lfg_frame &mv, const lfg_frame &out, float factor, bool intended, const InterpTables &tb, InterpRoute *route = nullptr);
 hipError_t launch_interpolate_multi(hipStream_t s, const lfg_frame &prev, const lfg_frame &curr, const lfg_frame &mv,
                                     const lfg_frame *const *outs, const float *factors, int count, bool intended,
-                                    const InterpTables &tb);
+                                    const InterpTables &tb, InterpRoute *route = nullptr);
+bool interpolate_reject_ok(const lfg_frame &prev, const lfg_frame &curr, const lfg_frame &mv, const lfg_frame *const *outs, int count,
+                           bool intended, const InterpTables &tb);
 size_t pyramid_workspace_bytes(uint32_t width, uint32_t height, int levels, PyramidLayout *layout);
 hipError_t launch_motion_pyramid(hipStream_t s, const lfg_frame &prev, const lfg_frame &curr, const lfg_frame &mv,
                                  int levels, int coarseRadius, int refineRadius, uint8_t *workspace, const PyramidLayout &layout);
```

New measurement: 4004 frames/s (median of 6 runs). 1.7% higher.
